# zongh5a/MDF-Net

Measured on AMD Instinct MI355X. Metric: views/sec at DTU 1600x1200x5-view x4-scale, higher is better.
Workload: dtype f32; 1 GPU; DTU eval 1600x1184 (1600x1200 cropped as load/dtueval.py:34), 5 views, 3 cost-volume stages + x2 refine = 4 output scales, hypotheses (48,24,8), batch 1 per rank, seeded random weights (pth/dtu_29.pth is not available offline); parallelism=views sharded over 1 rank(s), no collective

## Files before the change

### include/mdfnet_hip.h

```cpp
#ifndef MDFNET_HIP_H
#define MDFNET_HIP_H

#include <stdint.h>

#ifdef __cplusplus
extern "C" {
#endif

#define MDF_ABI_VERSION 1

#define MDF_OK 0
#define MDF_EARG (-1)
#define MDF_EUNSUPPORTED (-2)
#define MDF_EHIP (-3)

#define MDF_FEA_NCHW 0
#define MDF_FEA_NHWC 1
#define MDF_VOL_NCDHW 0
#define MDF_VOL_NDHWC 1

#define MDF_MAX_SRC_VIEWS 16
#define MDF_MAX_FUSE_VIEWS 1024

int mdf_abi_version(void);
const char* mdf_last_error(void);
const char* mdf_last_launch(void);
int mdf_release_stream(void* stream);

int mdf_homo_warp_fwd(const float* src_fea, int fea_layout, const float* proj, const float* hypos,
                      int hypos_per_pixel, float* out, int out_layout, int B, int C, int D, int h, int w,
                      void* stream);

int mdf_warp_corner_indices(const float* proj, const float* hypos, int hypos_per_pixel, int32_t* x0y0,
                            int B, int D, int h, int w, void* stream);

int mdf_warp_aggregate_vec_fwd(const float* ref_fea, const float* const* src_feas, int fea_layout,
                               const float* proj, const float* hypos, int hypos_per_pixel,
                               const float* w_params, float* cost, int cost_layout, int B, int C, int G,
                               int D, int h, int w, int n_src, void* stream);

int mdf_warp_aggregate_var_fwd(const float* ref_fea, const float* const* src_feas, int fea_layout,
                               const float* proj, const float* hypos, int hypos_per_pixel, float* cost,
                               int cost_layout, int B, int C, int D, int h, int w, int n_src, void* stream);

int mdf_conv3d_fwd(const float* x, const float* wpack, const float* alpha, const float* beta, const float* res,
                   float* y, int B, int Di, int Hi, int Wi, int Cin, int Cout, int stride, int transposed,
                   int relu, void* stream);

int64_t mdf_conv3d_packed_size(int Cin, int Cout);
int mdf_conv3d_pack_weights(const float* w, float* wpack, int Cin, int Cout, int transposed, void* stream);

int mdf_conv2d_fwd(const float* x, const float* wpack, const float* alpha, const float* beta, const float* res,
                   float res_scale, const float* res_up, float* y, int B, int H, int W, int Cin, int Cout, int ksize, int stride, int relu,
                   int planar_in, int pixel_shuffle2, void* stream);
int64_t mdf_conv_packed_size(int Cin, int Cout, int ntaps);
int mdf_conv_pack_weights(const float* w, float* wpack, int Cin, int Cout, int ntaps, void* stream);

int mdf_prob_softmax_regress_fwd(const float* x, const float* w, const float* hypos, int hypos_per_pixel,
                                 float* prob, float* depth, int B, int D, int h, int wd, int Cin, void* stream);
int mdf_prob_from_partials_fwd(const float* partials, const float* hypos, int hypos_per_pixel, float* prob, float* depth,
                               int B, int D, int h, int wd, void* stream);
int mdf_prob_fused_fwd(const float* x, const float* wpack, const float* hypos, int hypos_per_pixel, float* prob, float* depth,
                       int B, int D, int h, int wd, int Cin, void* stream);

int mdf_refine_tail_fwd(const float* x, const float* w1pack, const float* w2, const float* lo, const float* span, float* y,
                        int B, int H, int W, void* stream);

int mdf_conv2d_pair_fwd(const float* x, const float* w1pack, const float* alpha1, const float* beta1, const float* w2pack,
                        const float* alpha2, const float* beta2, float* y, int N, int H, int W, void* stream);

int mdf_conv1x1_heads_fwd(const float* x, int n_heads, const float* const* wpacks, const float* const* biases,
                          const float* const* res_ups, float* const* ys, const int* couts, int B, int H, int W, int Cin,
                          void* stream);

int mdf_refine_head_fwd(const float* depth, const float* lo, const float* span, const float* weight, float* y, int B, int H, int W,
                        void* stream);

int mdf_conv2d_res_pair_fwd(const float* x, const float* wa_pack, const float* wb_pack, float scale, float* y, int N, int H,
                            int W, void* stream);

int mdf_depth_regress_fwd(const float* prob, const float* hypos, int hypos_per_pixel, float* depth, int B, int D,
                          int h, int w, void* stream);

int mdf_confidence_fwd(const float* prob, float* conf, int64_t* idx_out, int B, int D, int h, int w, void* stream);
int mdf_confidence_up2_fwd(const float* prob, float* conf2, int B, int D, int h, int w, void* stream);
int mdf_range_affine_fwd(const float* x, const float* lo, const float* span, int mode, float* y, int B, long long n, void* stream);

int mdf_hypos_fit_fwd(int mode, const float* prob, const float* depth, const float* hypos, int hypos_per_pixel,
                      const float* fit_row, float* s_out, int B, int D, int h, int w, void* stream);
int mdf_hypos_from_fit_fwd(int mode, const float* s, const float* depth, const float* range, float log_thresh,
                           float* hypos_out, int B, int D_out, int h, int w, int upsample, void* stream);

int mdf_consistency_fuse_fwd(const float* depth_ref, const float* conf, const float* const* src_depths, const float* mats,
                             int n_src, int h, int w, float photo_threshold, int nconditions, float thre1, float thre2,
                             float* depth_avg, unsigned char* masks, unsigned short* view_masks, float* rep_out, void* stream);

long long mdf_consensus_fuse_workspace(int n, int h, int w);
int mdf_consensus_fuse_fwd(const float* depths, const unsigned char* colors, const float* cams, int n, int h, int w, float f,
                           float disp_thresh, int num_consistent, void* workspace, float* xyz, unsigned char* rgb,
                           long long capacity, int* view_counts, long long* total, void* stream);
int mdf_consensus_compact(void* workspace, int n, int h, int w, float* xyz, unsigned char* rgb, long long capacity, void* stream);

#define MDF_PCD_MAX_SOURCES 64
#define MDF_PCD_STEP_VIS1 1
#define MDF_PCD_STEP_FUSION 2
#define MDF_PCD_STEP_VIS2 3
#define MDF_PCD_STEP_AVE 4
#define MDF_PCD_STEP_VIS3 5
#define MDF_PCD_STEP_SEG 6
long long mdf_pcd_fuse_workspace(int n, int h, int w, int v);
int mdf_pcd_fuse_fwd(float* depths, unsigned char* masks, const float* cams, const int* srcs, int n, int h, int w, int v, int need,
                     int first_step, int last_step, void* workspace, int* view_counts, long long* total, void* stream);
int mdf_pcd_compact(const float* depths, const unsigned char* masks, const unsigned char* rgb, const float* cams, int n, int h,
                    int w, int v, void* workspace, float* xyz, unsigned char* rgb_out, float* dirs, long long capacity,
                    void* stream);

long long mdf_pts_index_workspace(long long n);
int mdf_pts_index_build(const double* pts, long long n, void* index, long long index_bytes, void* stream);
int mdf_pts_nn_dist(const void* index, long long n, long long index_bytes, const void* qindex, const double* queries, long long m,
                    long long qindex_bytes, const double* bb, double cap, double* dist, int* visits, void* stream);
long long mdf_pts_reduce_workspace(long long n);
int mdf_pts_reduce_count(const void* index, long long n, long long index_bytes, const int* rank, double dst, void* workspace,
                         long long ws_bytes, long long* edges, void* stream);
int mdf_pts_reduce(const void* index, long long n, long long index_bytes, const int* rank, double dst, void* workspace,
                   long long ws_bytes, int* csr, long long capacity, int resume, int max_rounds, unsigned char* keep, int* state,
                   void* stream);
int mdf_dtu_masks(const double* qdata, long long n, const unsigned char* obs_mask, int s1, int s2, int s3, const double* bb,
                  double res, unsigned char* in_mask, const double* qstl, long long m, const double* plane, unsigned char* above,
                  void* stream);


int mdf_bn_stats_fwd(const float* y, long long N, int C, int ngroups, double* sums, void* stream);
int mdf_bn_finalize_fwd(const double* sums, const float* gamma, const float* beta, float eps, float momentum, long long N,
                        int C, int ngroups, float* aux, float* running_mean, float* running_var,
                        long long* num_batches_tracked, int nslices, void* stream);
int mdf_bn_relu_apply_fwd(const float* y, const float* aux, const float* res, float* z, long long N, int C, int ngroups,
                          void* stream);
int mdf_bn_finalize_apply_fwd(const float* y, const double* sums, const float* gamma, const float* beta, float eps, float momentum,
                              const float* res, float* z, float* aux, float* running_mean, float* running_var,
                              long long* num_batches_tracked, long long N, int C, int ngroups, int nslices, void* stream);
int mdf_bn_relu_bwd_reduce(const float* dz, const float* y, const float* aux, long long N, int C, int ngroups, double* red,
                           void* stream);
int mdf_bn_relu_bwd(const float* dz, const float* y, const float* aux, const double* red, const float* gamma, long long N,
                    int C, int ngroups, float* dy, float* dgamma, float* dbeta, int nslices, void* stream);

int64_t mdf_conv3d_wgrad_workspace(int B, int Ds, int Hs, int Ws, int A, int Bc);
int mdf_conv3d_wgrad(const float* small_, const float* big, float* dw, float* workspace, int B, int Ds, int Hs, int Ws,
                     int A, int Bc, int stride, int accumulate, void* stream);
int64_t mdf_conv2d_wgrad_workspace(int B, int Hs, int Ws, int A, int Bc, int ksize);
int mdf_conv2d_wgrad(const float* small_, const float* big, float* dw, float* workspace, int B, int Hs, int Ws, int A, int Bc,
                     int ksize, int stride, int accumulate, void* stream);
int mdf_conv3d_wgrad_partial(const float* small_, const float* big, float* dw, float* workspace, int B, int Ds, int Hs, int Ws,
                             int A, int Bc, int stride, int* nslab_out, void* stream);
int mdf_conv2d_wgrad_partial(const float* small_, const float* big, float* dw, float* workspace, int B, int Hs, int Ws, int A, int Bc,
                             int ksize, int stride, int* nslab_out, void* stream);
int mdf_wgrad_sum_batch(const float* const* slabs, float* const* outs, const int* nslabs, const int* ns, int njobs, void* stream);
int mdf_wgrad_batch_begin(void);
int mdf_wgrad_batch_flush(void* stream);

int mdf_conv3d_train_fwd(const float* x, const float* wpack, const float* res, float* y, int B, int Di, int Hi, int Wi, int Cin,
                         int Cout, int stride, int transposed, int stat_mode, const float* stat_y, const float* stat_aux,
                         double* stat_out, int nslices, void* stream);
int mdf_conv2d_train_fwd(const float* x, const float* wpack, float* y, int B, int H, int W, int Cin_mem, int Cout, int ksize,
                         int stride, int planar_in, int stat_mode, const float* stat_y, const float* stat_aux, double* stat_out,
                         int nslices, int ngroups, void* stream);

int64_t mdf_pack_job_bytes(void);
int64_t mdf_pack_job_fill(void* jobs_host, int index, const float* src, float* dst, int is3d, int transposed, int mode,
                          int Cin, int Cout, int ntaps, int aux0, int aux1, int first_block);
int mdf_pack_batch(const void* jobs_dev, const int* block_job_dev, int nblocks, void* stream);

int mdf_upsample2_bilinear_bwd(const float* dfine, float* dcoarse, int B, int h, int w, int C, int accumulate, void* stream);

int mdf_prob_softmax_regress_bwd(const float* prob, const float* hypos, int hypos_per_pixel, const float* ddepth,
                                 const float* dprob, float* dlogit, int B, int D, int h, int w, void* stream);
int mdf_prob_conv_dgrad(const float* dlogit, const float* w, float* dx, int B, int D, int h, int wd, int C, void* stream);
int mdf_prob_conv_dgrad_stat(const float* dlogit, const float* w, float* dx, int B, int D, int h, int wd, int C, const float* stat_y,
                             const float* stat_aux, double* red, int nslices, void* stream);

int mdf_warp_aggregate_vec_train(int pass, const float* ref_fea, const float* const* src_feas, const float* proj,
                                 const float* hypos, int hypos_per_pixel, const float* par, const double* red_in,
                                 const float* dcost, float* cost, float* wsum, double* red_out, float* dref,
                                 float* const* dsrc, float* dcw, float* aux, int B, int C, int G, int D, int h, int w,
                                 int n_src, void* stream);
int mdf_aggregate_train_prepare(const float* cw, const float* w2, const float* b2, const float* gamma, long long n, int G,
                                int n_src, float* par, double* red, int nred, void* stream);
int mdf_aggregate_train_finalize(const double* red, const float* gamma, const float* beta, float eps, float momentum, long long n,
                                 int G, int n_src, float* par, float* running_mean, float* running_var,
                                 long long* num_batches_tracked, void* stream);
int mdf_aggregate_train_bwd_finalize(const float* dhalf, const double* red, int n_src, long long n_half, float* dsrc,
                                     float* dpar, const float* dref_acc, float* dref, long long n_ref, void* stream);

int mdf_masked_smooth_l1_reduce(const float* est, const float* gt, const void* floor_, int floor_f64, int floor_stride, int B,
                                long long per_batch, double* acc, void* stream);
int mdf_masked_smooth_l1_finalize(const double* acc, int nscales, float* loss, float* inv_count, void* stream);
int mdf_masked_smooth_l1_bwd(const float* est, const float* gt, const void* floor_, int floor_f64, int floor_stride, int B,
                             long long per_batch, const float* dloss, const float* inv_count, float* dest, void* stream);

int mdf_masked_smooth_l1_reduce_multi(const float* const* est, const float* const* gt, const long long* per_batch, int nscales,
                                      const void* floor_, int floor_f64, int floor_stride, int B, double* acc, void* stream);
int mdf_masked_smooth_l1_bwd_multi(const float* const* est, const float* const* gt, const long long* per_batch, int nscales,
                                   const void* floor_, int floor_f64, int floor_stride, int B, const float* dloss,
                                   const float* inv_count, float* const* dest, void* stream);

int mdf_fpn_compose_fwd(const float* O2, const float* O3, const float* L2, const float* b2, const float* L3, const float* b3,
                        int c2, int c3, int cm, float* comp, void* stream);
int mdf_fpn_compose_bwd(const float* O2, const float* O3, const float* L2, const float* b2, const float* L3, const float* b3,
                        const float* dA2, const float* dB3, const float* dA3, const float* W2, const float* W3,
                        const double* s2, const double* sc3, const double* s3, int c2, int c3, int cm, float* dO2, float* dO3,
                        float* dL2, float* dL3, float* db2, float* db3, void* stream);

int64_t mdf_adam_job_bytes(void);
int64_t mdf_adam_job_fill(void* jobs_host, int index, float* param, long long offset, long long n, int first_block);
int mdf_adam_step(const void* jobs_dev, const int* block_job_dev, int nblocks, const float* grads, float* exp_avg,
                  float* exp_avg_sq, float lr, float beta1, float beta2, float eps, float weight_decay, long long step,
                  void* stream);
int mdf_adam_step_hyper(const void* jobs_dev, const int* block_job_dev, int nblocks, const float* grads, float* exp_avg,
                        float* exp_avg_sq, const float* hyper_dev, float beta1, float beta2, float eps, float weight_decay,
                        void* stream);

#ifdef __cplusplus
}
#endif
#endif
```

### mdf-net_amd/csrc/conv1x1.hip

```cpp
#include <cstdlib>
#include "common.h"

namespace {

typedef float f32x4 __attribute__((ext_vector_type(4)));

struct P1 {
  const float* x;
  const float* wpack;
  const float* alpha;
  const float* beta;
  const float* res;
  const float* res_up;
  float* y;
  float res_scale;
  int relu;
  int Ho, Wo;
  long long npx;
  int n_runs;
};

struct PixBase { int img, oh, ow; };
__device__ __forceinline__ PixBase pix_base(unsigned first_px, int Ho, int Wo) {
  const unsigned rr = first_px / (unsigned)Wo, img = rr / (unsigned)Ho;
  return PixBase{(int)img, (int)(rr - img * (unsigned)Ho), (int)(first_px - rr * (unsigned)Wo)};
}
__device__ __forceinline__ void pix_at(const PixBase& b, int delta, int Ho, int Wo, int& img, int& oh, int& ow) {
  img = b.img; oh = b.oh; ow = b.ow + delta;
  while (ow >= Wo) {
    ow -= Wo;
    if (++oh == Ho) { oh = 0; ++img; }
  }
}

template <int CIN, int COUT>
__global__ __launch_bounds__(256) void conv1x1_kernel(const P1 p) {
  constexpr int NCH = CIN / 16, NT = COUT / 16;
  constexpr int U = (8 / NCH) < 1 ? 1 : 8 / NCH;
  const int lane = threadIdx.x & 63, q = lane >> 4, n16 = lane & 15;
  const int wave_g = blockIdx.x * 4 + (threadIdx.x >> 6), n_waves = gridDim.x * 4;

  float wr[NCH][NT][4];
#pragma unroll
  for (int ch = 0; ch < NCH; ++ch)
#pragma unroll
    for (int nt = 0; nt < NT; ++nt) {
      const float4 v = *reinterpret_cast<const float4*>(p.wpack + ((size_t)(ch * NT + nt) * 64 + lane) * 4);
      wr[ch][nt][0] = v.x; wr[ch][nt][1] = v.y; wr[ch][nt][2] = v.z; wr[ch][nt][3] = v.w;
    }
  float al[NT][4], be[NT][4];
#pragma unroll
  for (int nt = 0; nt < NT; ++nt)
#pragma unroll
    for (int k = 0; k < 4; ++k) {
      const int c = nt * 16 + 4 * q + k;
      al[nt][k] = p.alpha ? p.alpha[c] : 1.f;
      be[nt][k] = p.beta ? p.beta[c] : 0.f;
    }

  for (int run = wave_g; run < p.n_runs; run += n_waves) {
    const long long px0 = (long long)run * (U * 16) + n16;
    float4 xb[U][NCH];
#pragma unroll
    for (int u = 0; u < U; ++u) {
      const long long px = px0 + u * 16;
#pragma unroll
      for (int ch = 0; ch < NCH; ++ch)
        xb[u][ch] = (px < p.npx) ? *reinterpret_cast<const float4*>(p.x + px * CIN + ch * 16 + 4 * q) : make_float4(0.f, 0.f, 0.f, 0.f);
    }
    PixBase pb{0, 0, 0};
    if (p.res_up) pb = pix_base((unsigned)run * (U * 16), p.Ho, p.Wo);
#pragma unroll
    for (int u = 0; u < U; ++u) {
      const long long px = px0 + u * 16;
      f32x4 acc[NT];
#pragma unroll
      for (int nt = 0; nt < NT; ++nt) acc[nt] = (f32x4){0.f, 0.f, 0.f, 0.f};
#pragma unroll
      for (int ch = 0; ch < NCH; ++ch) {
        const float b4[4] = {xb[u][ch].x, xb[u][ch].y, xb[u][ch].z, xb[u][ch].w};
#pragma unroll
        for (int s = 0; s < 4; ++s)
#pragma unroll
          for (int nt = 0; nt < NT; ++nt) acc[nt] = __builtin_amdgcn_mfma_f32_16x16x4f32(wr[ch][nt][s], b4[s], acc[nt], 0, 0, 0);
      }
      if (px >= p.npx) continue;
      int oh = 0, ow = 0, img = 0;
      if (p.res_up) pix_at(pb, u * 16 + n16, p.Ho, p.Wo, img, oh, ow);
#pragma unroll
      for (int nt = 0; nt < NT; ++nt) {
        const int c0 = nt * 16 + 4 * q;
        float o[4];
#pragma unroll
        for (int k = 0; k < 4; ++k) {
          o[k] = acc[nt][k] * al[nt][k] + be[nt][k];
          if (p.relu) o[k] = fmaxf(o[k], 0.f);
        }
        if (p.res_up) {
          const int Hh = p.Ho >> 1, Wh = p.Wo >> 1;
          float sy = ((float)oh + 0.5f) * 0.5f - 0.5f; sy = sy < 0.f ? 0.f : sy;
          float sx = ((float)ow + 0.5f) * 0.5f - 0.5f; sx = sx < 0.f ? 0.f : sx;
          const int y0 = (int)sy, x0 = (int)sx;
          const int y1 = y0 + (y0 < Hh - 1), x1 = x0 + (x0 < Wh - 1);
          const float ly1 = sy - (float)y0, ly0 = 1.f - ly1, lx1 = sx - (float)x0, lx0 = 1.f - lx1;
          const float* base = p.res_up + (size_t)img * Hh * Wh * COUT + c0;
          const float4 v00 = *reinterpret_cast<const float4*>(base + ((size_t)y0 * Wh + x0) * COUT);
          const float4 v01 = *reinterpret_cast<const float4*>(base + ((size_t)y0 * Wh + x1) * COUT);
          const float4 v10 = *reinterpret_cast<const float4*>(base + ((size_t)y1 * Wh + x0) * COUT);
          const float4 v11 = *reinterpret_cast<const float4*>(base + ((size_t)y1 * Wh + x1) * COUT);
          const float w00 = ly0 * lx0, w01 = ly0 * lx1, w10 = ly1 * lx0, w11 = ly1 * lx1;
          o[0] = __fmaf_rn(w11, v11.x, __fmaf_rn(w10, v10.x, __fmaf_rn(w00, v00.x, w01 * v01.x))) + o[0];
          o[1] = __fmaf_rn(w11, v11.y, __fmaf_rn(w10, v10.y, __fmaf_rn(w00, v00.y, w01 * v01.y))) + o[1];
          o[2] = __fmaf_rn(w11, v11.z, __fmaf_rn(w10, v10.z, __fmaf_rn(w00, v00.z, w01 * v01.z))) + o[2];
          o[3] = __fmaf_rn(w11, v11.w, __fmaf_rn(w10, v10.w, __fmaf_rn(w00, v00.w, w01 * v01.w))) + o[3];
        }
        const size_t oi = (size_t)px * COUT + c0;
        if (p.res) {
          const float4 rv = *reinterpret_cast<const float4*>(p.res + oi);
          o[0] = rv.x + o[0] * p.res_scale; o[1] = rv.y + o[1] * p.res_scale;
          o[2] = rv.z + o[2] * p.res_scale; o[3] = rv.w + o[3] * p.res_scale;
        }
        *reinterpret_cast<float4*>(p.y + oi) = make_float4(o[0], o[1], o[2], o[3]);
      }
    }
  }
}

struct P1M {
  const float* x;
  const float* wpack[3];
  const float* beta[3];
  const float* res_up[3];
  float* y[3];
  int Ho, Wo;
  long long npx;
  int n_runs;
};

template <int CIN, int C0, int C1, int C2, int U>
__global__ __launch_bounds__(256) void conv1x1_heads_kernel(const P1M p) {
  constexpr int NCH = CIN / 16;
  constexpr int N0 = C0 / 16, N1 = C1 / 16, N2 = C2 / 16, NT = N0 + N1 + N2;
  const int lane = threadIdx.x & 63, q = lane >> 4, n16 = lane & 15;
  const int wave_g = blockIdx.x * 4 + (threadIdx.x >> 6), n_waves = gridDim.x * 4;
  auto head_of = [](int nt) { return nt < N0 ? 0 : (nt < N0 + N1 ? 1 : 2); };
  auto first_of = [](int h) { return h == 0 ? 0 : (h == 1 ? N0 : N0 + N1); };
  auto cout_of = [](int h) { return h == 0 ? C0 : (h == 1 ? C1 : C2); };

  constexpr bool WLDS = (NCH * NT * 4 > 64);
  __shared__ __attribute__((aligned(16))) float wsm[WLDS ? NCH * NT * 64 * 4 : 4];
  float wr[WLDS ? 1 : NCH][WLDS ? 1 : NT][4];
  float be[NT][4];
#pragma unroll
  for (int nt = 0; nt < NT; ++nt) {
    const int h = head_of(nt), lt = nt - first_of(h), nth = cout_of(h) / 16;
#pragma unroll
    for (int ch = 0; ch < NCH; ++ch) {
      if constexpr (WLDS) {
        if (threadIdx.x < 64)
          *reinterpret_cast<float4*>(wsm + ((ch * NT + nt) * 64 + lane) * 4) = *reinterpret_cast<const float4*>(p.wpack[h] + ((size_t)(ch * nth + lt) * 64 + lane) * 4);
      } else {
        const float4 v = *reinterpret_cast<const float4*>(p.wpack[h] + ((size_t)(ch * nth + lt) * 64 + lane) * 4);
        wr[ch][nt][0] = v.x; wr[ch][nt][1] = v.y; wr[ch][nt][2] = v.z; wr[ch][nt][3] = v.w;
      }
    }
#pragma unroll
    for (int k = 0; k < 4; ++k) be[nt][k] = p.beta[h] ? p.beta[h][lt * 16 + 4 * q + k] : 0.f;
  }
  if constexpr (WLDS) __syncthreads();

  for (int run = wave_g; run < p.n_runs; run += n_waves) {
    const long long px0 = (long long)run * (U * 16) + n16;
    float4 xb[U][NCH];
#pragma unroll
    for (int u = 0; u < U; ++u) {
      const long long px = px0 + u * 16;
#pragma unroll
      for (int ch = 0; ch < NCH; ++ch)
        xb[u][ch] = (px < p.npx) ? *reinterpret_cast<const float4*>(p.x + px * CIN + ch * 16 + 4 * q) : make_float4(0.f, 0.f, 0.f, 0.f);
    }
    const PixBase pb = pix_base((unsigned)run * (U * 16), p.Ho, p.Wo);
#pragma unroll
    for (int u = 0; u < U; ++u) {
      const long long px = px0 + u * 16;
      f32x4 acc[NT];
#pragma unroll
      for (int nt = 0; nt < NT; ++nt) acc[nt] = (f32x4){0.f, 0.f, 0.f, 0.f};
#pragma unroll
      for (int ch = 0; ch < NCH; ++ch) {
        const float b4[4] = {xb[u][ch].x, xb[u][ch].y, xb[u][ch].z, xb[u][ch].w};
        if constexpr (WLDS) {
          asm volatile("" ::: "memory");
#pragma unroll
          for (int nt = 0; nt < NT; ++nt) {
            const float4 wv = *reinterpret_cast<const float4*>(wsm + ((ch * NT + nt) * 64 + lane) * 4);
            const float w4[4] = {wv.x, wv.y, wv.z, wv.w};
#pragma unroll
            for (int s = 0; s < 4; ++s) acc[nt] = __builtin_amdgcn_mfma_f32_16x16x4f32(w4[s], b4[s], acc[nt], 0, 0, 0);
          }
        } else {
#pragma unroll
          for (int s = 0; s < 4; ++s)
#pragma unroll
            for (int nt = 0; nt < NT; ++nt) acc[nt] = __builtin_amdgcn_mfma_f32_16x16x4f32(wr[ch][nt][s], b4[s], acc[nt], 0, 0, 0);
        }
      }
      if (px >= p.npx) continue;
      int img, oh, ow;
      pix_at(pb, u * 16 + n16, p.Ho, p.Wo, img, oh, ow);
      const int Hh = p.Ho >> 1, Wh = p.Wo >> 1;
      float sy = ((float)oh + 0.5f) * 0.5f - 0.5f; sy = sy < 0.f ? 0.f : sy;
      float sx = ((float)ow + 0.5f) * 0.5f - 0.5f; sx = sx < 0.f ? 0.f : sx;
      const int y0 = (int)sy, x0 = (int)sx;
      const int y1 = y0 + (y0 < Hh - 1), x1 = x0 + (x0 < Wh - 1);
      const float ly1 = sy - (float)y0, ly0 = 1.f - ly1, lx1 = sx - (float)x0, lx0 = 1.f - lx1;
      const float w00 = ly0 * lx0, w01 = ly0 * lx1, w10 = ly1 * lx0, w11 = ly1 * lx1;
#pragma unroll
      for (int nt = 0; nt < NT; ++nt) {
        const int h = head_of(nt), co = cout_of(h), c0 = (nt - first_of(h)) * 16 + 4 * q;
        float o[4];
#pragma unroll
        for (int k = 0; k < 4; ++k) o[k] = acc[nt][k] * 1.0f + be[nt][k];
        if (p.res_up[h]) {
          const float* base = p.res_up[h] + (size_t)img * Hh * Wh * co + c0;
          const float4 v00 = *reinterpret_cast<const float4*>(base + ((size_t)y0 * Wh + x0) * co);
          const float4 v01 = *reinterpret_cast<const float4*>(base + ((size_t)y0 * Wh + x1) * co);
          const float4 v10 = *reinterpret_cast<const float4*>(base + ((size_t)y1 * Wh + x0) * co);
          const float4 v11 = *reinterpret_cast<const float4*>(base + ((size_t)y1 * Wh + x1) * co);
          o[0] = __fmaf_rn(w11, v11.x, __fmaf_rn(w10, v10.x, __fmaf_rn(w00, v00.x, w01 * v01.x))) + o[0];
          o[1] = __fmaf_rn(w11, v11.y, __fmaf_rn(w10, v10.y, __fmaf_rn(w00, v00.y, w01 * v01.y))) + o[1];
          o[2] = __fmaf_rn(w11, v11.z, __fmaf_rn(w10, v10.z, __fmaf_rn(w00, v00.z, w01 * v01.z))) + o[2];
          o[3] = __fmaf_rn(w11, v11.w, __fmaf_rn(w10, v10.w, __fmaf_rn(w00, v00.w, w01 * v01.w))) + o[3];
        }
        *reinterpret_cast<float4*>(p.y[h] + (size_t)px * co + c0) = make_float4(o[0], o[1], o[2], o[3]);
      }
    }
  }
}

template <int CIN, int C0, int C1, int C2, int U>
int launch_heads(P1M& p, hipStream_t st) {
  const long long runs = (p.npx + U * 16 - 1) / (U * 16);
  if (runs > 0x7fffffff) return mdf::fail(MDF_EARG, "conv1x1 heads: too many pixels");
  p.n_runs = (int)runs;
  long long blocks = (runs + 3) / 4;
  if (blocks > 256 * 8) blocks = 256 * 8;
  hipLaunchKernelGGL((conv1x1_heads_kernel<CIN, C0, C1, C2, U>), dim3((unsigned)blocks), dim3(256), 0, st, p);
  return mdf::check_launch("conv1x1_heads_kernel");
}

template <int CIN, int COUT>
int launch_1x1(P1& p, hipStream_t st) {
  constexpr int NCH = CIN / 16;
  constexpr int U = (8 / NCH) < 1 ? 1 : 8 / NCH;
  const long long runs = (p.npx + U * 16 - 1) / (U * 16);
  if (runs > 0x7fffffff) return mdf::fail(MDF_EARG, "conv1x1: too many pixels");
  p.n_runs = (int)runs;
  long long blocks = (runs + 3) / 4;
  int cap = 256 * 8;
  if (const char* e = getenv("MDF_CONV1X1_BLOCKS")) { if (atoi(e) > 0) cap = atoi(e); }
  if (blocks > cap) blocks = cap;
  hipLaunchKernelGGL((conv1x1_kernel<CIN, COUT>), dim3((unsigned)blocks), dim3(256), 0, st, p);
  return mdf::check_launch("conv1x1_kernel");
}

}

#define C1_CASE(ci, co) \
  if (Cin == ci && Cout == co) return launch_1x1<ci, co>(p, (hipStream_t)stream);

int mdf_conv1x1_dispatch(const float* x, const float* wpack, const float* alpha, const float* beta, const float* res, float res_scale,
                         const float* res_up, float* y, int B, int H, int W, int Cin, int Cout, int relu, void* stream) {
  if (const char* e = getenv("MDF_CONV1X1")) { if (atoi(e) == 0) return MDF_EUNSUPPORTED; }
  P1 p{};
  p.x = x; p.wpack = wpack; p.alpha = alpha; p.beta = beta; p.res = res; p.res_up = res_up; p.y = y;
  p.res_scale = res_scale; p.relu = relu; p.Ho = H; p.Wo = W; p.npx = (long long)B * H * W;
  if (p.npx >= (1ll << 31) - 256) return MDF_EUNSUPPORTED;
  C1_CASE(16, 16) C1_CASE(16, 32) C1_CASE(16, 64) C1_CASE(32, 16) C1_CASE(32, 32) C1_CASE(32, 64)
  return MDF_EUNSUPPORTED;
}

extern "C" int mdf_conv1x1_heads_fwd(const float* x, int n_heads, const float* const* wpacks, const float* const* biases,
                                     const float* const* res_ups, float* const* ys, const int* couts, int B, int H, int W, int Cin,
                                     void* stream) {
  MDF_REQUIRE(x && wpacks && biases && res_ups && ys && couts, "null pointer argument");
  MDF_REQUIRE(n_heads == 2 || n_heads == 3, "n_heads=%d not in {2,3}", n_heads);
  MDF_REQUIRE(B > 0 && H > 0 && W > 0, "bad shape");
  P1M p{};
  p.x = x; p.Ho = H; p.Wo = W; p.npx = (long long)B * H * W;
  bool any_up = false;
  for (int h = 0; h < n_heads; ++h) {
    MDF_REQUIRE(wpacks[h] && ys[h], "head %d: null weights or output", h);
    p.wpack[h] = wpacks[h]; p.beta[h] = biases[h]; p.res_up[h] = res_ups[h]; p.y[h] = ys[h];
    any_up = any_up || res_ups[h];
    MDF_REQUIRE((long long)p.npx * couts[h] < (1ll << 31) && (long long)p.npx * Cin < (1ll << 31), "map too large for 32-bit offsets");
  }
  MDF_REQUIRE(!any_up || (H % 2 == 0 && W % 2 == 0), "upsample-add needs even H and W");
  hipStream_t st = (hipStream_t)stream;
  if (Cin == 64 && n_heads == 3 && couts[0] == 64 && couts[1] == 32 && couts[2] == 16) return launch_heads<64, 64, 32, 16, 1>(p, st);
  if (Cin == 32 && n_heads == 2 && couts[0] == 32 && couts[1] == 16) return launch_heads<32, 32, 16, 0, 1>(p, st);
  return mdf::fail(MDF_EUNSUPPORTED, "conv1x1 heads: Cin=%d with %d heads is not built (64 -> 64/32/16, 32 -> 32/16)", Cin, n_heads);
}
```

### mdf-net_amd/csrc/warp_aggregate.hip

```cpp
#include <cstdlib>
#include "warp_common.h"

namespace {

enum Mode { kWarp = 0, kVec = 1, kVar = 2 };

struct Params {
  const float* ref;
  const float* src[MDF_MAX_SRC_VIEWS];
  const float* proj;
  const float* hypos;
  const float* wpar;
  float* out;
  Geom g;
  int B, D, n_src, hypos_per_pixel, out_ndhwc, dchunk, nblk_x;
};

template <int C, int MODE>
__global__ __launch_bounds__(kThreads) void warp_kernel(const Params p) {
  constexpr int LPP = C / 4;
  constexpr int PPB = kThreads / LPP;
  extern __shared__ __attribute__((aligned(16))) char smem[];
  TapEntry* tab = reinterpret_cast<TapEntry*>(smem);

  const int hw = p.g.h * p.g.w;
  const int b = blockIdx.y;
  const PixTile<PPB> pt((int)mdf::xcd_remap(blockIdx.x, p.nblk_x), p.g.w);
  const int tid = threadIdx.x;
  const int pl = tid / LPP;
  const int sub = tid % LPP;
  bool live;
  const int pix = pt.pix(pl, p.g.w, p.g.h, live);
  const int G = C / 2;

  float r[4] = {0.f, 0.f, 0.f, 0.f};
  float cw0 = 0.f, cw1 = 0.f, alpha = 0.f, beta = 0.f, w2 = 0.f, b2 = 0.f;
  if (MODE != kWarp) {
    const float4 rv = *reinterpret_cast<const float4*>(p.ref + ((size_t)b * hw + pix) * C + 4 * sub);
    if (MODE == kVec) {
      softmax2(rv.x, rv.y, r[0], r[1]);
      softmax2(rv.z, rv.w, r[2], r[3]);
      r[0] -= r[1];
      r[2] -= r[3];
      cw0 = p.wpar[2 * sub];
      cw1 = p.wpar[2 * sub + 1];
      alpha = p.wpar[G];
      beta = p.wpar[G + 1];
      w2 = p.wpar[G + 2];
      b2 = p.wpar[G + 3];
    } else {
      r[0] = rv.x; r[1] = rv.y; r[2] = rv.z; r[3] = rv.w;
    }
  }
  const size_t map_stride = (size_t)hw * C;
  const unsigned lane_b = 16u * (unsigned)sub;

  const int npair = PPB * p.n_src;
  const bool fixed_pair = (kThreads % npair) == 0;
  const int pa_pair = tid % npair, pa_grp = tid / npair, pa_ngrp = kThreads / npair;
  const int pa_pl = pa_pair % PPB, pa_v = pa_pair / PPB;
  bool pa_live;
  const int pa_pix = pt.pix(pa_pl, p.g.w, p.g.h, pa_live);
  PixelRay ray{};
  if (fixed_pair) {
    const int yy = pa_pix / p.g.w, xx = pa_pix - yy * p.g.w;
    ray = warp_ray(p.proj + ((size_t)pa_v * p.B + b) * 12, (float)xx, (float)yy);
  }

  for (int d0 = 0; d0 < p.D; d0 += p.dchunk) {
    const int nd = min(p.dchunk, p.D - d0);
    if (fixed_pair) {
      for (int ed = pa_grp; ed < nd; ed += pa_ngrp) {
        const int d = d0 + ed;
        const float dep = p.hypos_per_pixel ? p.hypos[((size_t)b * p.D + d) * hw + pa_pix] : p.hypos[(size_t)b * p.D + d];
        float ix, iy;
        warp_position_ray(ray, dep, p.g, ix, iy);
        TapEntry t;
        make_taps(ix, iy, p.g, C, t);
        tab[(ed * p.n_src + pa_v) * PPB + pa_pl] = t;
      }
    } else {
      const int nent = nd * p.n_src * PPB;
      for (int e = tid; e < nent; e += kThreads) {
        const int epl = e % PPB;
        const int ev = (e / PPB) % p.n_src;
        const int ed = e / (PPB * p.n_src);
        bool elive;
        const int epix = pt.pix(epl, p.g.w, p.g.h, elive);
        const int yy = epix / p.g.w, xx = epix - yy * p.g.w;
        const float* m = p.proj + ((size_t)ev * p.B + b) * 12;
        const int d = d0 + ed;
        const float dep = p.hypos_per_pixel ? p.hypos[((size_t)b * p.D + d) * hw + epix] : p.hypos[(size_t)b * p.D + d];
        float ix, iy;
        warp_position(m, (float)xx, (float)yy, dep, p.g, ix, iy);
        TapEntry t;
        make_taps(ix, iy, p.g, C, t);
        tab[e] = t;
      }
    }
    __syncthreads();
    for (int dd = 0; dd < nd; ++dd) {
      const int d = d0 + dd;
      float acc[4] = {0.f, 0.f, 0.f, 0.f};
      float acc2[4] = {0.f, 0.f, 0.f, 0.f};
      float wsum = 0.f;
      if (MODE == kVar) {
#pragma unroll
        for (int k = 0; k < 4; ++k) { acc[k] = r[k]; acc2[k] = r[k] * r[k]; }
      }
      for (int v = 0; v < p.n_src; ++v) {
        const TapEntry t = tab[(dd * p.n_src + v) * PPB + pl];
        const char* sb = reinterpret_cast<const char*>(p.src[v] + (size_t)b * map_stride);
        const float4 nw = *reinterpret_cast<const float4*>(sb + ((unsigned)t.off[0] * 4u + lane_b));
        const float4 ne = *reinterpret_cast<const float4*>(sb + ((unsigned)t.off[1] * 4u + lane_b));
        const float4 sw = *reinterpret_cast<const float4*>(sb + ((unsigned)t.off[2] * 4u + lane_b));
        const float4 se = *reinterpret_cast<const float4*>(sb + ((unsigned)t.off[3] * 4u + lane_b));
        float val[4];
        val[0] = __fmaf_rn(se.x, t.wt[3], __fmaf_rn(sw.x, t.wt[2], __fmaf_rn(ne.x, t.wt[1], __fmul_rn(nw.x, t.wt[0]))));
        val[1] = __fmaf_rn(se.y, t.wt[3], __fmaf_rn(sw.y, t.wt[2], __fmaf_rn(ne.y, t.wt[1], __fmul_rn(nw.y, t.wt[0]))));
        val[2] = __fmaf_rn(se.z, t.wt[3], __fmaf_rn(sw.z, t.wt[2], __fmaf_rn(ne.z, t.wt[1], __fmul_rn(nw.z, t.wt[0]))));
        val[3] = __fmaf_rn(se.w, t.wt[3], __fmaf_rn(sw.w, t.wt[2], __fmaf_rn(ne.w, t.wt[1], __fmul_rn(nw.w, t.wt[0]))));
        if (MODE == kWarp) {
#pragma unroll
          for (int k = 0; k < 4; ++k) acc[k] = val[k];
        } else if (MODE == kVec) {
          const float sim0 = __fmaf_rn(softmax2_p0(val[0], val[1]), r[0], r[1]);
          const float sim1 = __fmaf_rn(softmax2_p0(val[2], val[3]), r[2], r[3]);
          const float z = pixel_sum<LPP>(__fmaf_rn(cw0, sim0, cw1 * sim1));
          const float u = __fmaf_rn(fmaxf(__fmaf_rn(z, alpha, beta), 0.0f), w2, b2);
          const float wv = __builtin_amdgcn_rcpf(1.0f + __builtin_amdgcn_exp2f(-u * kLog2e));
          wsum += wv;
          acc[0] += wv * sim0;
          acc[1] += wv * sim1;
        } else {
          const float mx = pixel_max<LPP>(fmaxf(fmaxf(val[0], val[1]), fmaxf(val[2], val[3])));
          float e[4];
#pragma unroll
          for (int k = 0; k < 4; ++k) e[k] = expf(val[k] - mx);
          const float den = pixel_sum<LPP>((e[0] + e[1]) + (e[2] + e[3]));
#pragma unroll
          for (int k = 0; k < 4; ++k) {
            const float pr = e[k] / den;
            acc[k] += pr;
            acc2[k] += pr * pr;
          }
        }
      }
      if (!live) continue;
      const size_t vox = ((size_t)b * p.D + d) * hw + pix;
      if (MODE == kVec) {
        const float o0 = acc[0] / wsum, o1 = acc[1] / wsum;
        if (p.out_ndhwc) {
          { typedef float f2v __attribute__((ext_vector_type(2))); f2v ov = {o0, o1}; __builtin_nontemporal_store(ov, reinterpret_cast<f2v*>(p.out + vox * G + 2 * sub)); }
        } else {
          const size_t cs = (size_t)p.D * hw;
          float* o = p.out + ((size_t)b * G * p.D + d) * hw + pix;
          o[(size_t)(2 * sub) * cs] = o0;
          o[(size_t)(2 * sub + 1) * cs] = o1;
        }
      } else {
        float o[4];
        if (MODE == kVar) {
          const float n = (float)(p.n_src + 1);
#pragma unroll
          for (int k = 0; k < 4; ++k) {
            const float mean = acc[k] / n;
            o[k] = acc2[k] / n - mean * mean;
          }
        } else {
#pragma unroll
          for (int k = 0; k < 4; ++k) o[k] = acc[k];
        }
        if (p.out_ndhwc) {
          *reinterpret_cast<float4*>(p.out + vox * C + 4 * sub) = make_float4(o[0], o[1], o[2], o[3]);
        } else {
          const size_t cs = (size_t)p.D * hw;
          float* op = p.out + ((size_t)b * C * p.D + d) * hw + pix;
#pragma unroll
          for (int k = 0; k < 4; ++k) op[(size_t)(4 * sub + k) * cs] = o[k];
        }
      }
    }
    __syncthreads();
  }
}

#ifndef MDF_VEC8_MIN_BLOCKS
#define MDF_VEC8_MIN_BLOCKS 1
#endif
#ifndef MDF_VEC8_TAB
#define MDF_VEC8_TAB 1024
#endif
template <int C>
__global__ __launch_bounds__(kThreads, MDF_VEC8_MIN_BLOCKS) void warp_vec8_kernel(const Params p) {
  constexpr int LPP = C / 8;
  constexpr int PPB = kThreads / LPP;
  constexpr int G = C / 2;
  extern __shared__ __attribute__((aligned(16))) char smem[];
  TapEntry* tab = reinterpret_cast<TapEntry*>(smem);
  const int hw = p.g.h * p.g.w;
  const int b = blockIdx.y;
  const PixTile<PPB> pt((int)mdf::xcd_remap(blockIdx.x, p.nblk_x), p.g.w);
  const int tid = threadIdx.x;
  const int pl = tid / LPP, sub = tid % LPP;
  bool live;
  const int pix = pt.pix(pl, p.g.w, p.g.h, live);

  float rd[2][2], r1[2][2], cw[2][2];
#pragma unroll
  for (int j = 0; j < 2; ++j) {
    const float4 rv = *reinterpret_cast<const float4*>(p.ref + ((size_t)b * hw + pix) * C + 8 * sub + 4 * j);
    float a0, a1, b0, b1;
    softmax2(rv.x, rv.y, a0, a1);
    softmax2(rv.z, rv.w, b0, b1);
    rd[j][0] = a0 - a1; r1[j][0] = a1;
    rd[j][1] = b0 - b1; r1[j][1] = b1;
    cw[j][0] = p.wpar[2 * (2 * sub + j)];
    cw[j][1] = p.wpar[2 * (2 * sub + j) + 1];
  }
  const float alpha = p.wpar[G], beta = p.wpar[G + 1], w2 = p.wpar[G + 2], b2 = p.wpar[G + 3];
  const size_t map_stride = (size_t)hw * C;
  const unsigned lane_b = 32u * (unsigned)sub;

  const int npair = PPB * p.n_src;
  const bool few = (npair <= kThreads) && (kThreads % npair) == 0;
  const bool two = (npair == 2 * kThreads);
  const int pa_ngrp = few ? kThreads / npair : 1, pa_grp = few ? tid / npair : 0;
  PixelRay ray[2];
  int pa_pl[2], pa_v[2], pa_pix[2];
#pragma unroll
  for (int k = 0; k < 2; ++k) {
    const int pair = (few ? tid % npair : tid) + k * kThreads;
    pa_pl[k] = pair % PPB; pa_v[k] = min(pair / PPB, p.n_src - 1);
    bool pa_live;
    pa_pix[k] = pt.pix(pa_pl[k], p.g.w, p.g.h, pa_live);
    const int yy = pa_pix[k] / p.g.w, xx = pa_pix[k] - yy * p.g.w;
    ray[k] = warp_ray(p.proj + ((size_t)pa_v[k] * p.B + b) * 12, (float)xx, (float)yy);
  }

  for (int d0 = 0; d0 < p.D; d0 += p.dchunk) {
    const int nd = min(p.dchunk, p.D - d0);
    if (few || two) {
#pragma unroll
      for (int k = 0; k < 2; ++k) {
        if (k == 1 && !two) break;
        for (int ed = pa_grp; ed < nd; ed += pa_ngrp) {
          const int d = d0 + ed;
          const float dep = p.hypos_per_pixel ? p.hypos[((size_t)b * p.D + d) * hw + pa_pix[k]] : p.hypos[(size_t)b * p.D + d];
          float ix, iy;
          warp_position_ray(ray[k], dep, p.g, ix, iy);
          TapEntry t;
          make_taps(ix, iy, p.g, C, t);
          tab[(ed * p.n_src + pa_v[k]) * PPB + pa_pl[k]] = t;
        }
      }
    } else {
      const int nent = nd * p.n_src * PPB;
      for (int e = tid; e < nent; e += kThreads) {
        const int epl = e % PPB;
        const int ev = (e / PPB) % p.n_src;
        const int ed = e / (PPB * p.n_src);
        bool elive;
        const int epix = pt.pix(epl, p.g.w, p.g.h, elive);
        const int yy = epix / p.g.w, xx = epix - yy * p.g.w;
        const float* m = p.proj + ((size_t)ev * p.B + b) * 12;
        const int d = d0 + ed;
        const float dep = p.hypos_per_pixel ? p.hypos[((size_t)b * p.D + d) * hw + epix] : p.hypos[(size_t)b * p.D + d];
        float ix, iy;
        warp_position(m, (float)xx, (float)yy, dep, p.g, ix, iy);
        TapEntry t;
        make_taps(ix, iy, p.g, C, t);
        tab[e] = t;
      }
    }
    __syncthreads();
    for (int dd = 0; dd < nd; ++dd) {
      float acc[2][2] = {{0.f, 0.f}, {0.f, 0.f}};
      float wsum = 0.f;
      for (int v = 0; v < p.n_src; ++v) {
        const TapEntry t = tab[(dd * p.n_src + v) * PPB + pl];
        const char* sb = reinterpret_cast<const char*>(p.src[v] + (size_t)b * map_stride);
        float sim[2][2], part[2];
#pragma unroll
        for (int j = 0; j < 2; ++j) {
          const unsigned lb = lane_b + 16u * j;
          const float4 nw = *reinterpret_cast<const float4*>(sb + ((unsigned)t.off[0] * 4u + lb));
          const float4 ne = *reinterpret_cast<const float4*>(sb + ((unsigned)t.off[1] * 4u + lb));
          const float4 sw = *reinterpret_cast<const float4*>(sb + ((unsigned)t.off[2] * 4u + lb));
          const float4 se = *reinterpret_cast<const float4*>(sb + ((unsigned)t.off[3] * 4u + lb));
          const float v0 = __fmaf_rn(se.x, t.wt[3], __fmaf_rn(sw.x, t.wt[2], __fmaf_rn(ne.x, t.wt[1], __fmul_rn(nw.x, t.wt[0]))));
          const float v1 = __fmaf_rn(se.y, t.wt[3], __fmaf_rn(sw.y, t.wt[2], __fmaf_rn(ne.y, t.wt[1], __fmul_rn(nw.y, t.wt[0]))));
          const float v2 = __fmaf_rn(se.z, t.wt[3], __fmaf_rn(sw.z, t.wt[2], __fmaf_rn(ne.z, t.wt[1], __fmul_rn(nw.z, t.wt[0]))));
          const float v3 = __fmaf_rn(se.w, t.wt[3], __fmaf_rn(sw.w, t.wt[2], __fmaf_rn(ne.w, t.wt[1], __fmul_rn(nw.w, t.wt[0]))));
          sim[j][0] = __fmaf_rn(softmax2_p0(v0, v1), rd[j][0], r1[j][0]);
          sim[j][1] = __fmaf_rn(softmax2_p0(v2, v3), rd[j][1], r1[j][1]);
          part[j] = __fmaf_rn(cw[j][0], sim[j][0], cw[j][1] * sim[j][1]);
        }
        const float z = pixel_sum<LPP>(part[0] + part[1]);
        const float u = __fmaf_rn(fmaxf(__fmaf_rn(z, alpha, beta), 0.0f), w2, b2);
        const float wv = __builtin_amdgcn_rcpf(1.0f + __builtin_amdgcn_exp2f(-u * kLog2e));
        wsum += wv;
#pragma unroll
        for (int j = 0; j < 2; ++j) {
          acc[j][0] += wv * sim[j][0];
          acc[j][1] += wv * sim[j][1];
        }
      }
      if (!live) continue;
      const size_t vox = ((size_t)b * p.D + d0 + dd) * hw + pix;
      const float o0 = acc[0][0] / wsum, o1 = acc[0][1] / wsum, o2 = acc[1][0] / wsum, o3 = acc[1][1] / wsum;
      if (p.out_ndhwc) {
        { typedef float f4v __attribute__((ext_vector_type(4))); f4v ov = {o0, o1, o2, o3}; __builtin_nontemporal_store(ov, reinterpret_cast<f4v*>(p.out + vox * G + 4 * sub)); }
      } else {
        const size_t cs = (size_t)p.D * hw;
        float* o = p.out + ((size_t)b * G * p.D + d0 + dd) * hw + pix;
        o[(size_t)(4 * sub) * cs] = o0;
        o[(size_t)(4 * sub + 1) * cs] = o1;
        o[(size_t)(4 * sub + 2) * cs] = o2;
        o[(size_t)(4 * sub + 3) * cs] = o3;
      }
    }
    __syncthreads();
  }
}

template <int C>
int launch_vec8(Params& p, hipStream_t st) {
  constexpr int ppb = kThreads / (C / 8);
  p.nblk_x = PixTile<ppb>::blocks(p.g.w, p.g.h);
  int dch = MDF_VEC8_TAB / (p.n_src * ppb);
  if (dch < 1) dch = 1;
  if (dch > p.D) dch = p.D;
  p.dchunk = dch;
  const size_t lds = (size_t)dch * p.n_src * ppb * sizeof(TapEntry);
  if (lds > 64 * 1024) return MDF_EUNSUPPORTED;
  hipLaunchKernelGGL((warp_vec8_kernel<C>), dim3(p.nblk_x, p.B), dim3(kThreads), lds, st, p);
  return mdf::check_launch("warp_vec8_kernel");
}

struct WinDesc {
  int off;
  int xmin, ymin, ww;
};

template <int C>
__global__ __launch_bounds__(kThreads) void warp_vec_win_kernel(const Params p, int pool_floats) {
  constexpr int LPP = C / 4;
  constexpr int PPB = kThreads / LPP;
  constexpr int G = C / 2;
  extern __shared__ __attribute__((aligned(16))) char smem[];
  TapXY* tab = reinterpret_cast<TapXY*>(smem);
  float* pool = reinterpret_cast<float*>(smem + (size_t)p.dchunk * p.n_src * PPB * sizeof(TapXY));
  __shared__ int bb[MDF_MAX_SRC_VIEWS][4];
  __shared__ WinDesc wd[MDF_MAX_SRC_VIEWS];

  const int hw = p.g.h * p.g.w;
  const int W = p.g.w;
  const int b = blockIdx.y;
  const int tile = (int)mdf::xcd_remap(blockIdx.x, p.nblk_x);
  const int pix0 = tile * PPB;
  const int tid = threadIdx.x;
  const int pl = tid / LPP, sub = tid % LPP;
  const int pix = min(pix0 + pl, hw - 1);
  const bool live = (pix0 + pl) < hw;

  float r[4];
  {
    const float4 rv = *reinterpret_cast<const float4*>(p.ref + ((size_t)b * hw + pix) * C + 4 * sub);
    softmax2(rv.x, rv.y, r[0], r[1]);
    softmax2(rv.z, rv.w, r[2], r[3]);
    r[0] -= r[1];
    r[2] -= r[3];
  }
  const float cw0 = p.wpar[2 * sub], cw1 = p.wpar[2 * sub + 1];
  const float alpha = p.wpar[G], beta = p.wpar[G + 1], w2 = p.wpar[G + 2], b2 = p.wpar[G + 3];
  const size_t map_stride = (size_t)hw * C;

  for (int d0 = 0; d0 < p.D; d0 += p.dchunk) {
    const int nd = min(p.dchunk, p.D - d0);
    if (tid < 4 * p.n_src) bb[tid >> 2][tid & 3] = (tid & 1) ? INT32_MIN : INT32_MAX;
    __syncthreads();
    const int nent = nd * p.n_src * PPB;
    for (int e = tid; e < nent; e += kThreads) {
      const int epl = e % PPB;
      const int ev = (e / PPB) % p.n_src;
      const int ed = e / (PPB * p.n_src);
      const int epix = min(pix0 + epl, hw - 1);
      const int yy = epix / W, xx = epix - yy * W;
      const float* m = p.proj + ((size_t)ev * p.B + b) * 12;
      const int d = d0 + ed;
      const float dep = p.hypos_per_pixel ? p.hypos[((size_t)b * p.D + d) * hw + epix] : p.hypos[(size_t)b * p.D + d];
      float ix, iy;
      warp_position(m, (float)xx, (float)yy, dep, p.g, ix, iy);
      TapXY t;
      tap_weights_corners(ix, iy, p.g, t.wt, t.xa, t.xb, t.ya, t.yb);
      tab[e] = t;
      atomicMin(&bb[ev][0], t.xa);
      atomicMax(&bb[ev][1], t.xb);
      atomicMin(&bb[ev][2], t.ya);
      atomicMax(&bb[ev][3], t.yb);
    }
    __syncthreads();
    if (tid == 0) {
      int used = 0;
      for (int v = 0; v < p.n_src; ++v) {
        const int ww = bb[v][1] - bb[v][0] + 1, wh = bb[v][3] - bb[v][2] + 1;
        const long long need = (long long)ww * wh * C;
        WinDesc w_;
        w_.xmin = bb[v][0]; w_.ymin = bb[v][2]; w_.ww = ww;
        if (need <= pool_floats - used) { w_.off = used; used += (int)need; } else { w_.off = -1; }
        wd[v] = w_;
      }
    }
    __syncthreads();
    for (int v = 0; v < p.n_src; ++v) {
      const WinDesc w_ = wd[v];
      if (w_.off < 0) continue;
      const int wh = bb[v][3] - bb[v][2] + 1;
      const int row4 = w_.ww * (C / 4);
      const float* sv = p.src[v] + (size_t)b * map_stride;
      for (int wy = 0; wy < wh; ++wy) {
        const float4* grow = reinterpret_cast<const float4*>(sv + ((size_t)(w_.ymin + wy) * W + w_.xmin) * C);
        float4* lrow = reinterpret_cast<float4*>(pool + w_.off) + wy * row4;
        for (int j = tid; j < row4; j += kThreads) lrow[j] = grow[j];
      }
    }
    __syncthreads();

    for (int dd = 0; dd < nd; ++dd) {
      float acc0 = 0.f, acc1 = 0.f, wsum = 0.f;
      for (int v = 0; v < p.n_src; ++v) {
        const TapXY t = tab[(dd * p.n_src + v) * PPB + pl];
        const WinDesc w_ = wd[v];
        float4 nw, ne, sw, se;
        if (w_.off >= 0) {
          const float* lp = pool + w_.off + 4 * sub;
          const int ra = (t.ya - w_.ymin) * w_.ww, rb = (t.yb - w_.ymin) * w_.ww, ca = t.xa - w_.xmin, cb = t.xb - w_.xmin;
          nw = *reinterpret_cast<const float4*>(lp + (ra + ca) * C);
          ne = *reinterpret_cast<const float4*>(lp + (ra + cb) * C);
          sw = *reinterpret_cast<const float4*>(lp + (rb + ca) * C);
          se = *reinterpret_cast<const float4*>(lp + (rb + cb) * C);
        } else {
          const float* sp = p.src[v] + (size_t)b * map_stride + 4 * sub;
          nw = *reinterpret_cast<const float4*>(sp + (size_t)(t.ya * W + t.xa) * C);
          ne = *reinterpret_cast<const float4*>(sp + (size_t)(t.ya * W + t.xb) * C);
          sw = *reinterpret_cast<const float4*>(sp + (size_t)(t.yb * W + t.xa) * C);
          se = *reinterpret_cast<const float4*>(sp + (size_t)(t.yb * W + t.xb) * C);
        }
        const float v0 = __fmaf_rn(se.x, t.wt[3], __fmaf_rn(sw.x, t.wt[2], __fmaf_rn(ne.x, t.wt[1], __fmul_rn(nw.x, t.wt[0]))));
        const float v1 = __fmaf_rn(se.y, t.wt[3], __fmaf_rn(sw.y, t.wt[2], __fmaf_rn(ne.y, t.wt[1], __fmul_rn(nw.y, t.wt[0]))));
        const float v2 = __fmaf_rn(se.z, t.wt[3], __fmaf_rn(sw.z, t.wt[2], __fmaf_rn(ne.z, t.wt[1], __fmul_rn(nw.z, t.wt[0]))));
        const float v3 = __fmaf_rn(se.w, t.wt[3], __fmaf_rn(sw.w, t.wt[2], __fmaf_rn(ne.w, t.wt[1], __fmul_rn(nw.w, t.wt[0]))));
        const float sim0 = __fmaf_rn(softmax2_p0(v0, v1), r[0], r[1]);
        const float sim1 = __fmaf_rn(softmax2_p0(v2, v3), r[2], r[3]);
        const float z = pixel_sum<LPP>(__fmaf_rn(cw0, sim0, cw1 * sim1));
        const float u = __fmaf_rn(fmaxf(__fmaf_rn(z, alpha, beta), 0.0f), w2, b2);
        const float wv = __builtin_amdgcn_rcpf(1.0f + __builtin_amdgcn_exp2f(-u * kLog2e));
        wsum += wv;
        acc0 += wv * sim0;
        acc1 += wv * sim1;
      }
      if (!live) continue;
      const size_t vox = ((size_t)b * p.D + d0 + dd) * hw + pix;
      const float o0 = acc0 / wsum, o1 = acc1 / wsum;
      if (p.out_ndhwc) {
        *reinterpret_cast<float2*>(p.out + vox * G + 2 * sub) = make_float2(o0, o1);
      } else {
        const size_t cs = (size_t)p.D * hw;
        float* o = p.out + ((size_t)b * G * p.D + d0 + dd) * hw + pix;
        o[(size_t)(2 * sub) * cs] = o0;
        o[(size_t)(2 * sub + 1) * cs] = o1;
      }
    }
    __syncthreads();
  }
}

template <int C>
int launch_win(Params& p, hipStream_t st) {
  constexpr int ppb = kThreads / (C / 4);
  const int hw = p.g.h * p.g.w;
  p.nblk_x = (hw + ppb - 1) / ppb;
  int dch = 512 / (p.n_src * ppb);
  if (const char* e = getenv("MDF_WARP_DCHUNK")) { if (atoi(e) > 0) dch = atoi(e); }
  if (dch < 1) dch = 1;
  if (dch > p.D) dch = p.D;
  p.dchunk = dch;
  int pool_kb = 64;
  if (const char* e = getenv("MDF_WARP_POOL_KB")) { if (atoi(e) > 0) pool_kb = atoi(e); }
  const size_t tab_bytes = (size_t)dch * p.n_src * ppb * sizeof(TapXY);
  const size_t lds = tab_bytes + (size_t)pool_kb * 1024;
  if (lds > 150 * 1024) return MDF_EUNSUPPORTED;
  static bool attr_done[64] = {};
  int dev_id = 0;
  (void)hipGetDevice(&dev_id);
  if (dev_id < 0 || dev_id >= 64 || !attr_done[dev_id]) {
    hipError_t e = hipFuncSetAttribute(reinterpret_cast<const void*>(&warp_vec_win_kernel<C>), hipFuncAttributeMaxDynamicSharedMemorySize, 150 * 1024);
    if (e != hipSuccess) return mdf::fail(MDF_EHIP, "hipFuncSetAttribute(dynamic LDS): %s", hipGetErrorString(e));
    if (dev_id >= 0 && dev_id < 64) attr_done[dev_id] = true;
  }
  hipLaunchKernelGGL((warp_vec_win_kernel<C>), dim3(p.nblk_x, p.B), dim3(kThreads), lds, st, p, pool_kb * 256);
  return mdf::check_launch("warp_vec_win_kernel");
}

__global__ void corner_index_kernel(const float* __restrict__ proj, const float* __restrict__ hypos, int per_pixel,
                                    int32_t* __restrict__ out, Geom g, int B, int D) {
  const int hw = g.h * g.w;
  const size_t n = (size_t)B * D * hw;
  for (size_t i = (size_t)blockIdx.x * blockDim.x + threadIdx.x; i < n; i += (size_t)gridDim.x * blockDim.x) {
    const int pix = (int)(i % hw);
    const int d = (int)((i / hw) % D);
    const int b = (int)(i / ((size_t)hw * D));
    const int yy = pix / g.w, xx = pix - yy * g.w;
    const float dep = per_pixel ? hypos[i] : hypos[(size_t)b * D + d];
    float ix, iy;
    warp_position(proj + (size_t)b * 12, (float)xx, (float)yy, dep, g, ix, iy);
    const float lim = 1073741824.0f;
    const bool fin = (fabsf(ix) <= 3.0e38f) && (fabsf(iy) <= 3.0e38f);
    int32_t x0 = INT32_MIN, y0 = INT32_MIN;
    if (fin) {
      x0 = (int32_t)fminf(fmaxf(floorf(ix), -lim), lim);
      y0 = (int32_t)fminf(fmaxf(floorf(iy), -lim), lim);
    }
    out[2 * i] = x0;
    out[2 * i + 1] = y0;
  }
}

template <int MODE>
int launch(Params& p, int C, hipStream_t st) {
  const int lpp = C / 4, ppb = kThreads / lpp;
  p.nblk_x = (C == 64) ? PixTile<16>::blocks(p.g.w, p.g.h) : (C == 32) ? PixTile<32>::blocks(p.g.w, p.g.h) : PixTile<64>::blocks(p.g.w, p.g.h);
  int dch = 512 / (p.n_src * ppb);
  if (dch < 1) dch = 1;
  if (dch > p.D) dch = p.D;
  p.dchunk = dch;
  const size_t lds = (size_t)dch * p.n_src * ppb * sizeof(TapEntry);
  dim3 grid(p.nblk_x, p.B), block(kThreads);
  switch (C) {
    case 64: hipLaunchKernelGGL((warp_kernel<64, MODE>), grid, block, lds, st, p); break;
    case 32: hipLaunchKernelGGL((warp_kernel<32, MODE>), grid, block, lds, st, p); break;
    case 16: hipLaunchKernelGGL((warp_kernel<16, MODE>), grid, block, lds, st, p); break;
    default: return mdf::fail(MDF_EUNSUPPORTED, "warp kernels are built for C in {16,32,64}, got %d", C);
  }
  return mdf::check_launch("warp_kernel");
}

int check_common(const void* a, const void* b, const void* c, const void* d, int fea_layout, int B, int C, int D, int h,
                 int w) {
  MDF_REQUIRE(a && b && c && d, "null pointer argument");
  MDF_REQUIRE(B > 0 && D > 0 && h > 1 && w > 1, "bad shape B=%d D=%d h=%d w=%d", B, D, h, w);
  MDF_REQUIRE((long long)h * w * C < (1ll << 30), "feature map too large for 32-bit byte offsets");
  if (fea_layout != MDF_FEA_NHWC)
    return mdf::fail(MDF_EUNSUPPORTED, "feature layout %d not supported (kernels gather NHWC taps)", fea_layout);
  if (C != 16 && C != 32 && C != 64)
    return mdf::fail(MDF_EUNSUPPORTED, "C=%d not supported (built for 16, 32, 64)", C);
  return MDF_OK;
}

}

extern "C" int mdf_homo_warp_fwd(const float* src_fea, int fea_layout, const float* proj, const float* hypos,
                                 int hypos_per_pixel, float* out, int out_layout, int B, int C, int D, int h, int w,
                                 void* stream) {
  if (int rc = check_common(src_fea, proj, hypos, out, fea_layout, B, C, D, h, w)) return rc;
  Params p{};
  p.src[0] = src_fea;
  p.proj = proj;
  p.hypos = hypos;
  p.out = out;
  p.g = make_geom(h, w);
  p.B = B; p.D = D; p.n_src = 1; p.hypos_per_pixel = hypos_per_pixel; p.out_ndhwc = (out_layout == MDF_VOL_NDHWC);
  return launch<kWarp>(p, C, (hipStream_t)stream);
}

extern "C" int mdf_warp_corner_indices(const float* proj, const float* hypos, int hypos_per_pixel, int32_t* x0y0,
                                       int B, int D, int h, int w, void* stream) {
  MDF_REQUIRE(proj && hypos && x0y0, "null pointer argument");
  MDF_REQUIRE(B > 0 && D > 0 && h > 1 && w > 1, "bad shape");
  const size_t n = (size_t)B * D * h * w;
  const int grid = (int)((n + 255) / 256 < 4096 ? (n + 255) / 256 : 4096);
  hipLaunchKernelGGL(corner_index_kernel, dim3(grid), dim3(256), 0, (hipStream_t)stream, proj, hypos, hypos_per_pixel,
                     x0y0, make_geom(h, w), B, D);
  return mdf::check_launch("corner_index_kernel");
}

extern "C" int mdf_warp_aggregate_vec_fwd(const float* ref_fea, const float* const* src_feas, int fea_layout,
                                          const float* proj, const float* hypos, int hypos_per_pixel,
                                          const float* w_params, float* cost, int cost_layout, int B, int C, int G,
                                          int D, int h, int w, int n_src, void* stream) {
  if (int rc = check_common(ref_fea, proj, hypos, cost, fea_layout, B, C, D, h, w)) return rc;
  MDF_REQUIRE(src_feas && w_params, "null pointer argument");
  MDF_REQUIRE(n_src >= 1 && n_src <= MDF_MAX_SRC_VIEWS, "n_src=%d out of range [1,%d]", n_src, MDF_MAX_SRC_VIEWS);
  if (G * 2 != C) return mdf::fail(MDF_EUNSUPPORTED, "only C/G == 2 is built (C=%d, G=%d)", C, G);
  Params p{};
  p.ref = ref_fea;
  for (int v = 0; v < n_src; ++v) {
    MDF_REQUIRE(src_feas[v], "src_feas[%d] is null", v);
    p.src[v] = src_feas[v];
  }
  p.proj = proj; p.hypos = hypos; p.wpar = w_params; p.out = cost;
  p.g = make_geom(h, w);
  p.B = B; p.D = D; p.n_src = n_src; p.hypos_per_pixel = hypos_per_pixel; p.out_ndhwc = (cost_layout == MDF_VOL_NDHWC);
  const char* we = getenv("MDF_WARP_WINDOW");
  if (we && atoi(we) != 0) {
    int rc = MDF_EUNSUPPORTED;
    if (C == 64) rc = launch_win<64>(p, (hipStream_t)stream);
    else if (C == 32) rc = launch_win<32>(p, (hipStream_t)stream);
    else if (C == 16) rc = launch_win<16>(p, (hipStream_t)stream);
    if (rc != MDF_EUNSUPPORTED) return rc;
  }
  {
    const char* e8 = getenv("MDF_WARP_VEC8");
    if (!e8 || atoi(e8) != 0) {
      int rc = MDF_EUNSUPPORTED;
      if (C == 64) rc = launch_vec8<64>(p, (hipStream_t)stream);
      else if (C == 32) rc = launch_vec8<32>(p, (hipStream_t)stream);
      else if (C == 16 && e8 && atoi(e8) == 2) rc = launch_vec8<16>(p, (hipStream_t)stream);
      if (rc != MDF_EUNSUPPORTED) return rc;
    }
  }
  return launch<kVec>(p, C, (hipStream_t)stream);
}

extern "C" int mdf_warp_aggregate_var_fwd(const float* ref_fea, const float* const* src_feas, int fea_layout,
                                          const float* proj, const float* hypos, int hypos_per_pixel, float* cost,
                                          int cost_layout, int B, int C, int D, int h, int w, int n_src, void* stream) {
  if (int rc = check_common(ref_fea, proj, hypos, cost, fea_layout, B, C, D, h, w)) return rc;
  MDF_REQUIRE(src_feas, "null pointer argument");
  MDF_REQUIRE(n_src >= 1 && n_src <= MDF_MAX_SRC_VIEWS, "n_src=%d out of range [1,%d]", n_src, MDF_MAX_SRC_VIEWS);
  Params p{};
  p.ref = ref_fea;
  for (int v = 0; v < n_src; ++v) {
    MDF_REQUIRE(src_feas[v], "src_feas[%d] is null", v);
    p.src[v] = src_feas[v];
  }
  p.proj = proj; p.hypos = hypos; p.out = cost;
  p.g = make_geom(h, w);
  p.B = B; p.D = D; p.n_src = n_src; p.hypos_per_pixel = hypos_per_pixel; p.out_ndhwc = (cost_layout == MDF_VOL_NDHWC);
  return launch<kVar>(p, C, (hipStream_t)stream);
}
```

### mdf-net_amd/mdfnet_hip/__init__.py

```python
import ctypes
import os
import threading

import torch

_PKG = os.path.dirname(os.path.abspath(__file__))
LIB_PATH = os.environ.get("MDF_HIP_LIB") or os.path.join(_PKG, "libmdfnet_hip.so")
ABI_VERSION = 1

_lib = None
_lock = threading.Lock()

c_fp = ctypes.c_void_p
c_int = ctypes.c_int
c_i64 = ctypes.c_int64

SIGNATURES = {
    "mdf_abi_version": (c_int, []),
    "mdf_last_error": (ctypes.c_char_p, []),
    "mdf_last_launch": (ctypes.c_char_p, []),
    "mdf_release_stream": (c_int, [c_fp]),
    "mdf_homo_warp_fwd": (c_int, [c_fp, c_int, c_fp, c_fp, c_int, c_fp, c_int] + [c_int] * 5 + [c_fp]),
    "mdf_warp_corner_indices": (c_int, [c_fp, c_fp, c_int, c_fp] + [c_int] * 4 + [c_fp]),
    "mdf_warp_aggregate_vec_fwd": (c_int, [c_fp, ctypes.POINTER(c_fp), c_int, c_fp, c_fp, c_int, c_fp, c_fp, c_int]
                                   + [c_int] * 7 + [c_fp]),
    "mdf_warp_aggregate_var_fwd": (c_int, [c_fp, ctypes.POINTER(c_fp), c_int, c_fp, c_fp, c_int, c_fp, c_int]
                                   + [c_int] * 6 + [c_fp]),
    "mdf_conv3d_fwd": (c_int, [c_fp] * 6 + [c_int] * 9 + [c_fp]),
    "mdf_conv3d_packed_size": (c_i64, [c_int, c_int]),
    "mdf_conv3d_pack_weights": (c_int, [c_fp, c_fp, c_int, c_int, c_int, c_fp]),
    "mdf_conv2d_fwd": (c_int, [c_fp] * 5 + [ctypes.c_float, c_fp, c_fp] + [c_int] * 10 + [c_fp]),
    "mdf_conv2d_pair_fwd": (c_int, [c_fp] * 8 + [c_int] * 3 + [c_fp]),
    "mdf_conv1x1_heads_fwd": (c_int, [c_fp, c_int, ctypes.POINTER(c_fp), ctypes.POINTER(c_fp), ctypes.POINTER(c_fp), ctypes.POINTER(c_fp),
                                      ctypes.POINTER(c_int)] + [c_int] * 4 + [c_fp]),
    "mdf_refine_head_fwd": (c_int, [c_fp] * 5 + [c_int] * 3 + [c_fp]),
    "mdf_conv2d_res_pair_fwd": (c_int, [c_fp] * 3 + [ctypes.c_float, c_fp] + [c_int] * 3 + [c_fp]),
    "mdf_refine_tail_fwd": (c_int, [c_fp] * 6 + [c_int] * 3 + [c_fp]),
    "mdf_conv_packed_size": (c_i64, [c_int, c_int, c_int]),
    "mdf_conv_pack_weights": (c_int, [c_fp, c_fp, c_int, c_int, c_int, c_fp]),
    "mdf_prob_softmax_regress_fwd": (c_int, [c_fp, c_fp, c_fp, c_int, c_fp, c_fp] + [c_int] * 5 + [c_fp]),
    "mdf_prob_from_partials_fwd": (c_int, [c_fp, c_fp, c_int, c_fp, c_fp] + [c_int] * 4 + [c_fp]),
    "mdf_prob_fused_fwd": (c_int, [c_fp, c_fp, c_fp, c_int, c_fp, c_fp] + [c_int] * 5 + [c_fp]),
    "mdf_depth_regress_fwd": (c_int, [c_fp, c_fp, c_int, c_fp] + [c_int] * 4 + [c_fp]),
    "mdf_confidence_fwd": (c_int, [c_fp, c_fp, c_fp] + [c_int] * 4 + [c_fp]),
    "mdf_confidence_up2_fwd": (c_int, [c_fp, c_fp] + [c_int] * 4 + [c_fp]),
    "mdf_range_affine_fwd": (c_int, [c_fp, c_fp, c_fp, c_int, c_fp, c_int, c_i64, c_fp]),
    "mdf_hypos_fit_fwd": (c_int, [c_int, c_fp, c_fp, c_fp, c_int, c_fp, c_fp] + [c_int] * 4 + [c_fp]),
    "mdf_consistency_fuse_fwd": (c_int, [c_fp, c_fp, ctypes.POINTER(c_fp), c_fp, c_int, c_int, c_int, ctypes.c_float, c_int,
                                         ctypes.c_float, ctypes.c_float, c_fp, c_fp, c_fp, c_fp, c_fp]),
    "mdf_consensus_fuse_workspace": (c_i64, [c_int, c_int, c_int]),
    "mdf_consensus_fuse_fwd": (c_int, [c_fp, c_fp, c_fp, c_int, c_int, c_int, ctypes.c_float, ctypes.c_float, c_int, c_fp, c_fp, c_fp,
                                       c_i64, c_fp, c_fp, c_fp]),
    "mdf_consensus_compact": (c_int, [c_fp, c_int, c_int, c_int, c_fp, c_fp, c_i64, c_fp]),
    "mdf_pcd_fuse_workspace": (c_i64, [c_int, c_int, c_int, c_int]),
    "mdf_pcd_fuse_fwd": (c_int, [c_fp, c_fp, c_fp, c_fp] + [c_int] * 7 + [c_fp, c_fp, c_fp, c_fp]),
    "mdf_pcd_compact": (c_int, [c_fp, c_fp, c_fp, c_fp] + [c_int] * 4 + [c_fp, c_fp, c_fp, c_fp, c_i64, c_fp]),
    "mdf_pts_index_workspace": (c_i64, [c_i64]),
    "mdf_pts_index_build": (c_int, [c_fp, c_i64, c_fp, c_i64, c_fp]),
    "mdf_pts_nn_dist": (c_int, [c_fp, c_i64, c_i64, c_fp, c_fp, c_i64, c_i64, ctypes.POINTER(ctypes.c_double), ctypes.c_double, c_fp,
                                c_fp, c_fp]),
    "mdf_pts_reduce_workspace": (c_i64, [c_i64]),
    "mdf_pts_reduce_count": (c_int, [c_fp, c_i64, c_i64, c_fp, ctypes.c_double, c_fp, c_i64, c_fp, c_fp]),
    "mdf_pts_reduce": (c_int, [c_fp, c_i64, c_i64, c_fp, ctypes.c_double, c_fp, c_i64, c_fp, c_i64, c_int, c_int, c_fp, c_fp, c_fp]),
    "mdf_dtu_masks": (c_int, [c_fp, c_i64, c_fp, c_int, c_int, c_int, ctypes.POINTER(ctypes.c_double), ctypes.c_double, c_fp, c_fp,
                              c_i64, ctypes.POINTER(ctypes.c_double), c_fp, c_fp]),
    "mdf_bn_stats_fwd": (c_int, [c_fp, c_i64, c_int, c_int, c_fp, c_fp]),
    "mdf_bn_finalize_fwd": (c_int, [c_fp, c_fp, c_fp, ctypes.c_float, ctypes.c_float, c_i64, c_int, c_int, c_fp, c_fp, c_fp, c_fp, c_int, c_fp]),
    "mdf_bn_relu_apply_fwd": (c_int, [c_fp, c_fp, c_fp, c_fp, c_i64, c_int, c_int, c_fp]),
    "mdf_bn_finalize_apply_fwd": (c_int, [c_fp, c_fp, c_fp, c_fp, ctypes.c_float, ctypes.c_float, c_fp, c_fp, c_fp, c_fp, c_fp, c_fp, c_i64, c_int, c_int, c_int, c_fp]),
    "mdf_bn_relu_bwd_reduce": (c_int, [c_fp, c_fp, c_fp, c_i64, c_int, c_int, c_fp, c_fp]),
    "mdf_bn_relu_bwd": (c_int, [c_fp, c_fp, c_fp, c_fp, c_fp, c_i64, c_int, c_int, c_fp, c_fp, c_fp, c_int, c_fp]),
    "mdf_conv3d_wgrad_workspace": (c_i64, [c_int] * 6),
    "mdf_conv3d_wgrad": (c_int, [c_fp] * 4 + [c_int] * 8 + [c_fp]),
    "mdf_conv3d_train_fwd": (c_int, [c_fp] * 4 + [c_int] * 9 + [c_fp] * 3 + [c_int, c_fp]),
    "mdf_conv2d_train_fwd": (c_int, [c_fp] * 3 + [c_int] * 9 + [c_fp] * 3 + [c_int, c_int, c_fp]),
    "mdf_conv3d_wgrad_partial": (c_int, [c_fp] * 4 + [c_int] * 7 + [ctypes.POINTER(c_int), c_fp]),
    "mdf_conv2d_wgrad_partial": (c_int, [c_fp] * 4 + [c_int] * 7 + [ctypes.POINTER(c_int), c_fp]),
    "mdf_wgrad_sum_batch": (c_int, [ctypes.POINTER(c_fp), ctypes.POINTER(c_fp), ctypes.POINTER(c_int), ctypes.POINTER(c_int), c_int, c_fp]),
    "mdf_wgrad_batch_begin": (c_int, []),
    "mdf_wgrad_batch_flush": (c_int, [c_fp]),
    "mdf_conv2d_wgrad_workspace": (c_i64, [c_int] * 6),
    "mdf_conv2d_wgrad": (c_int, [c_fp] * 4 + [c_int] * 8 + [c_fp]),
    "mdf_pack_job_bytes": (c_i64, []),
    "mdf_pack_job_fill": (c_i64, [c_fp, c_int, c_fp, c_fp] + [c_int] * 9),
    "mdf_pack_batch": (c_int, [c_fp, c_fp, c_int, c_fp]),
    "mdf_upsample2_bilinear_bwd": (c_int, [c_fp, c_fp] + [c_int] * 5 + [c_fp]),
    "mdf_prob_softmax_regress_bwd": (c_int, [c_fp, c_fp, c_int, c_fp, c_fp, c_fp] + [c_int] * 4 + [c_fp]),
    "mdf_prob_conv_dgrad": (c_int, [c_fp, c_fp, c_fp] + [c_int] * 5 + [c_fp]),
    "mdf_prob_conv_dgrad_stat": (c_int, [c_fp, c_fp, c_fp] + [c_int] * 5 + [c_fp, c_fp, c_fp, c_int, c_fp]),
    "mdf_warp_aggregate_vec_train": (c_int, [c_int, c_fp, ctypes.POINTER(c_fp), c_fp, c_fp, c_int, c_fp, c_fp, c_fp, c_fp, c_fp, c_fp,
                                             c_fp, ctypes.POINTER(c_fp), c_fp, c_fp] + [c_int] * 7 + [c_fp]),
    "mdf_aggregate_train_prepare": (c_int, [c_fp] * 4 + [c_i64, c_int, c_int, c_fp, c_fp, c_int, c_fp]),
    "mdf_aggregate_train_finalize": (c_int, [c_fp] * 3 + [ctypes.c_float, ctypes.c_float, c_i64, c_int, c_int] + [c_fp] * 5),
    "mdf_aggregate_train_bwd_finalize": (c_int, [c_fp, c_fp, c_int, c_i64, c_fp, c_fp, c_fp, c_fp, c_i64, c_fp]),
    "mdf_masked_smooth_l1_reduce": (c_int, [c_fp, c_fp, c_fp, c_int, c_int, c_int, c_i64, c_fp, c_fp]),
    "mdf_masked_smooth_l1_finalize": (c_int, [c_fp, c_int, c_fp, c_fp, c_fp]),
    "mdf_masked_smooth_l1_bwd": (c_int, [c_fp, c_fp, c_fp, c_int, c_int, c_int, c_i64, c_fp, c_fp, c_fp, c_fp]),
    "mdf_masked_smooth_l1_reduce_multi": (c_int, [ctypes.POINTER(c_fp), ctypes.POINTER(c_fp), ctypes.POINTER(c_i64), c_int, c_fp, c_int, c_int, c_int, c_fp, c_fp]),
    "mdf_masked_smooth_l1_bwd_multi": (c_int, [ctypes.POINTER(c_fp), ctypes.POINTER(c_fp), ctypes.POINTER(c_i64), c_int, c_fp, c_int, c_int, c_int, c_fp, c_fp,
                                               ctypes.POINTER(c_fp), c_fp]),
    "mdf_fpn_compose_fwd": (c_int, [c_fp] * 6 + [c_int] * 3 + [c_fp, c_fp]),
    "mdf_fpn_compose_bwd": (c_int, [c_fp] * 14 + [c_int] * 3 + [c_fp] * 7),
    "mdf_adam_job_bytes": (c_i64, []),
    "mdf_adam_job_fill": (c_i64, [c_fp, c_int, c_fp, c_i64, c_i64, c_int]),
    "mdf_adam_step": (c_int, [c_fp, c_fp, c_int, c_fp, c_fp, c_fp] + [ctypes.c_float] * 5 + [c_i64, c_fp]),
    "mdf_adam_step_hyper": (c_int, [c_fp, c_fp, c_int, c_fp, c_fp, c_fp, c_fp] + [ctypes.c_float] * 4 + [c_fp]),
    "mdf_hypos_from_fit_fwd": (c_int, [c_int, c_fp, c_fp, c_fp, ctypes.c_float, c_fp] + [c_int] * 5 + [c_fp]),
}


class MdfHipError(RuntimeError):
    pass


def lib():
    global _lib
    if _lib is None:
        with _lock:
            if _lib is None:
                if not os.path.exists(LIB_PATH):
                    raise MdfHipError(
                        f"{LIB_PATH} not found: the HIP extension is not built and there is no fallback path. "
                        "Run `python -m mdfnet_hip.build` (needs hipcc, --offload-arch=gfx950).")
                h = ctypes.CDLL(LIB_PATH)
                for name, (res, args) in SIGNATURES.items():
                    fn = getattr(h, name)
                    fn.restype = res
                    fn.argtypes = args
                if h.mdf_abi_version() != ABI_VERSION:
                    raise MdfHipError(f"ABI version mismatch: library {h.mdf_abi_version()}, binding {ABI_VERSION}")
                _lib = h
    return _lib


def check(rc, what):
    if rc != 0:
        msg = lib().mdf_last_error().decode("utf-8", "replace")
        raise MdfHipError(f"{what} failed with code {rc}: {msg}")


def pcd_fuse(*args, **kwargs):
    from .ops import pcd_fuse as _pcd_fuse
    return _pcd_fuse(*args, **kwargs)


def dtu_eval_scan(*args, **kwargs):
    from .ops import dtu_eval_scan as _dtu_eval_scan
    return _dtu_eval_scan(*args, **kwargs)
```

### mdf-net_amd/mdfnet_hip/kernel_families.py

```python
import re

MFMA_CONV = "mfma_conv"
WARP = "warp_aggregate"
WARP_TRAIN = "aggregate_train_passes"
WARP_SCATTER = "aggregate_scatter"
WGRAD = "wgrad"
BN = "batchnorm_train"
PROB = "prob_head"
HEADS = "heads"
FILTER = "consistency_filter"
POINT_EVAL = "point_eval"
CONTROL = "control"

KERNEL_FAMILY = {
    "conv_lds_kernel": MFMA_CONV, "conv3d_kernel": MFMA_CONV, "conv3d_wlds_kernel": MFMA_CONV, "convtr_all_kernel": MFMA_CONV, "convtr_cls_kernel": MFMA_CONV, "conv_pair_kernel": MFMA_CONV, "conv_pair_valu_kernel": MFMA_CONV,
    "conv1x1_kernel": MFMA_CONV, "conv1x1_heads_kernel": MFMA_CONV, "refine_tail_kernel": MFMA_CONV, "prob_fused_kernel": MFMA_CONV, "res_pair_kernel": MFMA_CONV,
    "wino3d_kernel": MFMA_CONV, "wino2d_kernel": MFMA_CONV,
    "pack_weights_kernel": CONTROL, "pack_batch_kernel": CONTROL,
    "warp_kernel": WARP, "warp_vec8_kernel": WARP, "warp_vec_win_kernel": WARP, "corner_index_kernel": WARP,
    "warp_train_kernel": WARP_TRAIN, "warp_bwd_kernel": WARP_SCATTER,
    "agg_prepare_kernel": CONTROL, "agg_finalize_kernel": CONTROL, "agg_bwd_finalize_kernel": WARP_SCATTER,
    "wgrad_kernel": WGRAD, "wgrad_a1_kernel": WGRAD, "wgrad_a1_valu_kernel": WGRAD, "wgrad2d_kernel": WGRAD,
    "wgrad_lds_kernel": WGRAD, "wgrad_lds_batch_kernel": WGRAD, "slab_sum_kernel": WGRAD, "slab_sum_batch_kernel": WGRAD,
    "bn_reduce_kernel": BN, "bn_finalize_kernel": BN, "bn_relu_apply_kernel": BN, "bn_finalize_apply_kernel": BN,
    "bn_relu_bwd_kernel": BN,
    "prob_head_kernel": PROB, "prob_head_tiled_kernel": PROB, "prob_from_partials_kernel": PROB,
    "softmax_regress_bwd_kernel": PROB, "prob_conv_dgrad_kernel": PROB, "upsample2_bwd_kernel": PROB,
    "depth_regress_kernel": HEADS, "confidence_kernel": HEADS, "confidence_up2_kernel": HEADS, "range_affine_kernel": HEADS,
    "hypos_fit_kernel": HEADS, "hypos_from_fit_kernel": HEADS, "refine_head_kernel": HEADS, "fpn_compose_fwd_kernel": HEADS, "fpn_compose_bwd_kernel": HEADS,
    "consistency_fuse_kernel": FILTER,
    "consensus_fuse_kernel": FILTER, "consensus_scan_kernel": FILTER, "consensus_compact_kernel": FILTER,
    "pcd_reproj_kernel": FILTER, "pcd_cand_count_kernel": FILTER, "pcd_cand_place_kernel": FILTER, "pcd_select_kernel": FILTER, "pcd_select_big_kernel": FILTER, "pcd_bin_sum_kernel": FILTER, "pcd_bin_offsets_kernel": FILTER,
    "pcd_seg_init_kernel": FILTER, "pcd_seg_hook_kernel": FILTER, "pcd_seg_count_kernel": FILTER, "pcd_seg_apply_kernel": FILTER,
    "pcd_count_kernel": FILTER, "pcd_scan_kernel": FILTER, "pcd_compact_kernel": FILTER,
    "pts_bbox_kernel": POINT_EVAL, "pts_bbox_final_kernel": POINT_EVAL, "pts_morton_kernel": POINT_EVAL, "pts_sort_hist_kernel": POINT_EVAL,
    "pts_sort_scan_kernel": POINT_EVAL, "pts_sort_scatter_kernel": POINT_EVAL, "pts_gather_kernel": POINT_EVAL, "pts_leaf_kernel": POINT_EVAL,
    "pts_node_kernel": POINT_EVAL, "pts_nn_kernel": POINT_EVAL, "pts_rank_kernel": POINT_EVAL, "pts_radius_kernel": POINT_EVAL,
    "pts_reduce_init_kernel": POINT_EVAL, "pts_reduce_round_kernel": POINT_EVAL, "pts_reduce_step_kernel": POINT_EVAL,
    "pts_reduce_keep_kernel": POINT_EVAL, "pts_dtu_masks_kernel": POINT_EVAL,
    "masked_smooth_l1_reduce_kernel": CONTROL, "masked_smooth_l1_finalize_kernel": CONTROL, "masked_smooth_l1_bwd_kernel": CONTROL,
    "masked_smooth_l1_reduce_multi_kernel": CONTROL, "masked_smooth_l1_bwd_multi_kernel": CONTROL, "adam_step_kernel": CONTROL,
}

def function_name(rocprof_name):
    s = rocprof_name.strip()
    if s.startswith("void "):
        s = s[5:]
    s = s.replace("(anonymous namespace)::", "")
    head = re.split(r"[<(]", s, maxsplit=1)[0]
    return head.split("::")[-1].strip()


def family(rocprof_name):
    return KERNEL_FAMILY.get(function_name(rocprof_name))


def is_ours(rocprof_name):
    return function_name(rocprof_name) in KERNEL_FAMILY


def globals_in_sources(csrc_dir):
    import os
    names = {}
    for f in sorted(os.listdir(csrc_dir)):
        if not f.endswith(".hip"):
            continue
        text = open(os.path.join(csrc_dir, f)).read()
        for m in re.finditer(r"__global__\b[\s\S]*?\bvoid\s+([A-Za-z_][A-Za-z_0-9]*)\s*\(", text):
            names.setdefault(m.group(1), f)
    return names


def fetch_size_factor(rocprof_name):
    return 2.0
```

### mdf-net_amd/mdfnet_hip/ops.py

```python
import ctypes
import os
import threading

import torch

from . import check, lib

FEA_NHWC = 1
VOL_NCDHW, VOL_NDHWC = 0, 1

_prof = None


def profile_begin():
    global _prof
    _prof = []


def profile_end():
    global _prof
    recs, _prof = _prof, None
    torch.cuda.synchronize()
    return [(n, tag, e0.elapsed_time(e1), work) for n, tag, e0, e1, work in recs]


_counts = None


def count_begin():
    global _counts
    _counts = {}


def count_end():
    global _counts
    c, _counts = _counts, None
    return c


def _abi(name, args, tag="", work=None):
    fn = getattr(lib(), name)
    if _counts is not None:
        _counts[name] = _counts.get(name, 0) + 1
    if _prof is None:
        check(fn(*args), name)
        return
    e0, e1 = torch.cuda.Event(enable_timing=True), torch.cuda.Event(enable_timing=True)
    e0.record()
    check(fn(*args), name)
    e1.record()
    _prof.append((name, tag, e0, e1, dict(work or {}, kernel=lib().mdf_last_launch().decode())))


class _single_thread:

    def __enter__(self):
        self.n = torch.get_num_threads()
        if self.n > 1:
            torch.set_num_threads(1)

    def __exit__(self, *a):
        if self.n > 1:
            torch.set_num_threads(self.n)


_raw_stream = getattr(torch._C, "_cuda_getCurrentRawStream", None)


def _stream(t):
    if _raw_stream is not None:
        return ctypes.c_void_p(_raw_stream(t.device.index if t.device.index is not None else torch.cuda.current_device()))
    return ctypes.c_void_p(torch.cuda.current_stream(t.device).cuda_stream)


def _need_gpu(*ts):
    for t in ts:
        if t is not None and not t.is_cuda:
            raise RuntimeError("mdfnet_hip ops run on an MI355X only (got a CPU tensor); there is no CPU fallback")


def _f32c(t):
    return t if (t.dtype == torch.float32 and t.is_contiguous()) else t.float().contiguous()


def nhwc(t):
    return t.float().contiguous(memory_format=torch.channels_last)


_recorded = threading.local()


class recorded_host_values:
    def __init__(self, projs=None, fit_row=None, log_thresh=None, cams=None):
        self.v = {"projs": list(projs or []), "cams": list(cams or []), "fit_row": fit_row, "log_thresh": log_thresh or {}}

    def __enter__(self):
        _recorded.v = self.v
        return self

    def __exit__(self, *exc):
        _recorded.v = None


def recorded(kind, key=None):
    v = getattr(_recorded, "v", None)
    if v is None:
        return None
    if kind in ("projs", "cams"):
        return torch.as_tensor(v[kind].pop(0)).float().contiguous() if v[kind] else None
    if kind == "log_thresh":
        return v["log_thresh"].get(key)
    return None if v[kind] is None else torch.as_tensor(v[kind]).float().contiguous()


def relative_projections(ref_proj, src_projs):
    pinned = recorded("projs")
    if pinned is not None:
        return pinned
    ref = ref_proj.detach().to("cpu", torch.float32)
    with _single_thread():
        inv = torch.inverse(ref)
        rows = [torch.matmul(sp.detach().to("cpu", torch.float32), inv)[:, :3, :4].reshape(-1, 12) for sp in src_projs]
        return torch.stack(rows, 0).contiguous()


def _hypos_arg(hypos, h, w):
    per_pixel = int(hypos.shape[-1] != 1 or hypos.shape[-2] != 1)
    if per_pixel and (hypos.shape[-2] != h or hypos.shape[-1] != w):
        raise ValueError(f"depth_hypos {tuple(hypos.shape)} does not match feature size {(h, w)}")
    return _f32c(hypos), per_pixel


def homo_warp(src_fea, proj12, depth_hypos):
    _need_gpu(src_fea, proj12, depth_hypos)
    b, c, h, w = src_fea.shape
    d = depth_hypos.shape[1]
    fea = nhwc(src_fea)
    hyp, pp = _hypos_arg(depth_hypos, h, w)
    out = torch.empty((b, c, d, h, w), device=src_fea.device, dtype=torch.float32)
    _abi("mdf_homo_warp_fwd", (fea.data_ptr(), FEA_NHWC, _f32c(proj12).data_ptr(), hyp.data_ptr(), pp,
                                  out.data_ptr(), VOL_NCDHW, b, c, d, h, w, _stream(out),))
    return out


def warp_corner_indices(proj12, depth_hypos, h, w):
    _need_gpu(proj12, depth_hypos)
    b, d = depth_hypos.shape[:2]
    hyp, pp = _hypos_arg(depth_hypos, h, w)
    out = torch.empty((b, d, h, w, 2), device=proj12.device, dtype=torch.int32)
    _abi("mdf_warp_corner_indices", (_f32c(proj12).data_ptr(), hyp.data_ptr(), pp, out.data_ptr(), b, d, h, w,
                                        _stream(out),))
    return out


def _src_array(srcs):
    arr = (ctypes.c_void_p * len(srcs))(*[s.data_ptr() for s in srcs])
    return arr


def warp_aggregate_vec(features, proj, depth_hypos, w_params, ngroups, channels_last=True):
    _need_gpu(*features, proj, depth_hypos, w_params)
    feas = [nhwc(f) for f in features]
    b, c, h, w = feas[0].shape
    d = depth_hypos.shape[1]
    hyp, pp = _hypos_arg(depth_hypos, h, w)
    g = ngroups
    dev = feas[0].device
    if channels_last:
        mem = torch.empty((b, d, h, w, g), device=dev, dtype=torch.float32)
        cost = mem.permute(0, 4, 1, 2, 3)
    else:
        mem = cost = torch.empty((b, g, d, h, w), device=dev, dtype=torch.float32)
    srcs = feas[1:]
    _abi("mdf_warp_aggregate_vec_fwd", (feas[0].data_ptr(), _src_array(srcs), FEA_NHWC, _f32c(proj).data_ptr(),
                                           hyp.data_ptr(), pp, _f32c(w_params).data_ptr(), mem.data_ptr(),
                                           VOL_NDHWC if channels_last else VOL_NCDHW, b, c, g, d, h, w, len(srcs),
                                           _stream(mem),), tag=f"C{c}G{g}D{d} {w}x{h} V{len(feas)}",
         work={"bytes": 4.0 * b * (len(feas) * c * h * w + hyp.numel() / b + g * d * h * w),
               "bound": "hbm"})
    return cost


def warp_aggregate_var(features, proj, depth_hypos, channels_last=False):
    _need_gpu(*features, proj, depth_hypos)
    feas = [nhwc(f) for f in features]
    b, c, h, w = feas[0].shape
    d = depth_hypos.shape[1]
    hyp, pp = _hypos_arg(depth_hypos, h, w)
    dev = feas[0].device
    if channels_last:
        mem = torch.empty((b, d, h, w, c), device=dev, dtype=torch.float32)
        cost = mem.permute(0, 4, 1, 2, 3)
    else:
        mem = cost = torch.empty((b, c, d, h, w), device=dev, dtype=torch.float32)
    srcs = feas[1:]
    _abi("mdf_warp_aggregate_var_fwd", (feas[0].data_ptr(), _src_array(srcs), FEA_NHWC, _f32c(proj).data_ptr(),
                                           hyp.data_ptr(), pp, mem.data_ptr(),
                                           VOL_NDHWC if channels_last else VOL_NCDHW, b, c, d, h, w, len(srcs),
                                           _stream(mem),))
    return cost


def fold_view_weight(p, ngroups, prefix="depth_weight."):
    cw = p[prefix + "0.conv.weight"].reshape(ngroups).float()
    invstd = 1.0 / torch.sqrt(p[prefix + "0.bn.running_var"].float() + 1e-5)
    alpha = p[prefix + "0.bn.weight"].float() * invstd
    beta = p[prefix + "0.bn.bias"].float() - p[prefix + "0.bn.running_mean"].float() * alpha
    return torch.cat([cw, alpha.reshape(1), beta.reshape(1), p[prefix + "1.weight"].reshape(1).float(),
                      p[prefix + "1.bias"].reshape(1).float()]).contiguous()


def depth_regress(prob, depth_hypos):
    _need_gpu(prob, depth_hypos)
    b, d, h, w = prob.shape
    hyp, pp = _hypos_arg(depth_hypos, h, w)
    prob = _f32c(prob)
    out = torch.empty((b, h, w), device=prob.device, dtype=torch.float32)
    _abi("mdf_depth_regress_fwd", (prob.data_ptr(), hyp.data_ptr(), pp, out.data_ptr(), b, d, h, w, _stream(out),))
    return out


def confidence(prob, return_index=False):
    _need_gpu(prob)
    b, d, h, w = prob.shape
    prob = _f32c(prob)
    out = torch.empty((b, h, w), device=prob.device, dtype=torch.float32)
    idx = torch.empty((b, h, w), device=prob.device, dtype=torch.int64) if return_index else None
    _abi("mdf_confidence_fwd", (prob.data_ptr(), out.data_ptr(), idx.data_ptr() if return_index else None,
                                   b, d, h, w, _stream(out),))
    return (out, idx) if return_index else out


def confidence_up2(prob):
    _need_gpu(prob)
    b, d, h, w = prob.shape
    prob = _f32c(prob)
    out = torch.empty((b, 2 * h, 2 * w), device=prob.device, dtype=torch.float32)
    _abi("mdf_confidence_up2_fwd", (prob.data_ptr(), out.data_ptr(), b, d, h, w, _stream(out),))
    return out


def range_affine(x, lo, span, mode):
    _need_gpu(x, lo, span)
    x = _f32c(x)
    y = torch.empty_like(x)
    b = x.shape[0]
    lo_c, span_c = _f32c(lo), _f32c(span)
    _abi("mdf_range_affine_fwd", (x.data_ptr(), lo_c.data_ptr(), span_c.data_ptr(), mode, y.data_ptr(), b, x.numel() // b, _stream(y),))
    return y


_fit_row_cache = {}


def gauss1_fit_row(depth_hypos):
    pinned = recorded("fit_row")
    if pinned is not None:
        return pinned
    hyp = depth_hypos.detach().to("cpu", torch.float32)
    b, d = hyp.shape[:2]
    key = (b, d, hyp.numpy().tobytes())
    row = _fit_row_cache.get(key)
    if row is None:
        with _single_thread():
            rep = hyp.reshape(b, d, 1, 1).repeat(1, 1, 2, 2)
            x = torch.stack([rep ** 2, rep, torch.ones_like(rep)], dim=-1).permute(0, 2, 3, 1, 4)
            xt = x.transpose(-1, -2)
            row = torch.matmul(torch.inverse(torch.matmul(xt, x)), xt)[:, 0, 0, 0, :].contiguous()
        if len(_fit_row_cache) > 256:
            _fit_row_cache.clear()
        _fit_row_cache[key] = row
    return row


def hypos_fit(mode, prob, depth, depth_hypos, fit_row=None):
    _need_gpu(prob)
    b, d, h, w = prob.shape
    prob = _f32c(prob)
    hyp, pp = _hypos_arg(depth_hypos, h, w)
    out = torch.empty((b, h, w), device=prob.device, dtype=torch.float32)
    _abi("mdf_hypos_fit_fwd", (mode, prob.data_ptr(), None if depth is None else _f32c(depth).data_ptr(),
                                  hyp.data_ptr(), pp, None if fit_row is None else _f32c(fit_row).data_ptr(),
                                  out.data_ptr(), b, d, h, w, _stream(out),))
    return out


def hypos_from_fit(mode, s, depth, depth_range_f32, log_thresh, ndepths, upsample=True):
    _need_gpu(s, depth, depth_range_f32)
    b, h, w = s.shape
    ho, wo = (2 * h, 2 * w) if upsample else (h, w)
    out = torch.empty((b, ndepths, ho, wo), device=s.device, dtype=torch.float32)
    _abi("mdf_hypos_from_fit_fwd", (mode, _f32c(s).data_ptr(), _f32c(depth).data_ptr(),
                                       _f32c(depth_range_f32).data_ptr(), ctypes.c_float(log_thresh), out.data_ptr(),
                                       b, ndepths, h, w, int(upsample), _stream(out),))
    return out


def to_ndhwc(t):
    cl = t.permute(0, 2, 3, 4, 1)
    return cl if (cl.is_contiguous() and cl.dtype == torch.float32) else cl.float().contiguous()


def from_ndhwc(cl):
    return cl.permute(0, 4, 1, 2, 3)


def pack_conv3d_weight(w, transposed=False):
    _need_gpu(w)
    cin, cout = (w.shape[0], w.shape[1]) if transposed else (w.shape[1], w.shape[0])
    n = lib().mdf_conv3d_packed_size(cin, cout)
    out = torch.empty((n,), device=w.device, dtype=torch.float32)
    _abi("mdf_conv3d_pack_weights", (_f32c(w.detach()).data_ptr(), out.data_ptr(), cin, cout, int(transposed),
                                        _stream(out),))
    return out


def conv3d_ndhwc(x, wpack, cin, cout, stride=1, transposed=False, alpha=None, beta=None, relu=False, res=None):
    _need_gpu(x, wpack)
    b, d, h, w, c = x.shape
    assert c == cin and x.is_contiguous()
    if transposed:
        do, ho, wo = 2 * d, 2 * h, 2 * w
    elif stride == 2:
        do, ho, wo = (d - 1) // 2 + 1, (h - 1) // 2 + 1, (w - 1) // 2 + 1
    else:
        do, ho, wo = d, h, w
    y = torch.empty((b, do, ho, wo, cout), device=x.device, dtype=torch.float32)
    if res is not None:
        assert res.shape == y.shape and res.is_contiguous()
    _abi("mdf_conv3d_fwd", (x.data_ptr(), wpack.data_ptr(), None if alpha is None else alpha.data_ptr(),
                               None if beta is None else beta.data_ptr(), None if res is None else res.data_ptr(),
                               y.data_ptr(), b, d, h, w, cin, cout, stride, int(transposed), int(relu), _stream(y),),
         tag=f"{cin}->{cout} {'T' if transposed else 's%d' % stride} {d}x{h}x{w}",
         work={"flops": 2.0 * 27 * cin * cout * b * (d * h * w if transposed else do * ho * wo),
               "bytes": 4.0 * (x.numel() + y.numel() * (2 if res is not None else 1)), "bound": "mfma"})
    return y


STAT_SLICES = 16


def conv3d_train(x, wpack, cin, cout, stride, transposed, res, stat_mode, stat_out, stat_y=None, stat_aux=None):
    _need_gpu(x, wpack, stat_out)
    b, d, h, w, c = x.shape
    assert c == cin and x.is_contiguous()
    if transposed:
        do, ho, wo = 2 * d, 2 * h, 2 * w
    elif stride == 2:
        do, ho, wo = (d - 1) // 2 + 1, (h - 1) // 2 + 1, (w - 1) // 2 + 1
    else:
        do, ho, wo = d, h, w
    y = torch.empty((b, do, ho, wo, cout), device=x.device, dtype=torch.float32)
    if res is not None:
        assert res.shape == y.shape and res.is_contiguous()
    if stat_mode == 2:
        assert stat_y.shape == y.shape and stat_y.is_contiguous() and stat_aux.numel() == 4 * cout
    nslices = stat_out.numel() // (2 * cout)
    assert stat_out.numel() == nslices * 2 * cout and stat_out.dtype == torch.float64
    _abi("mdf_conv3d_train_fwd", (x.data_ptr(), wpack.data_ptr(), None if res is None else res.data_ptr(), y.data_ptr(), b, d, h, w, cin, cout,
                                  stride, int(transposed), stat_mode, None if stat_y is None else stat_y.data_ptr(),
                                  None if stat_aux is None else stat_aux.data_ptr(), stat_out.data_ptr(), nslices, _stream(y)),
         tag=f"{cin}->{cout} {'T' if transposed else 's%d' % stride} {d}x{h}x{w} +sums{stat_mode}",
         work={"flops": 2.0 * 27 * cin * cout * b * (d * h * w if transposed else do * ho * wo),
               "bytes": 4.0 * (x.numel() + y.numel() * (1 + (res is not None) + (stat_mode == 2))), "bound": "mfma"})
    return y


def conv2d_train(x, wpack, cin, cout, ksize, stride, planar_in, stat_mode, stat_out, ngroups, stat_y=None, stat_aux=None):
    _need_gpu(x, wpack, stat_out)
    if planar_in:
        b, c, h, w = x.shape
    else:
        b, h, w, c = x.shape
    assert c == cin and x.is_contiguous() and b % ngroups == 0
    pad = (ksize - 1) // 2
    ho, wo = (h + 2 * pad - ksize) // stride + 1, (w + 2 * pad - ksize) // stride + 1
    y = torch.empty((b, ho, wo, cout), device=x.device, dtype=torch.float32)
    if stat_mode == 2:
        assert stat_y.shape == y.shape and stat_y.is_contiguous() and stat_aux.numel() == ngroups * 4 * cout
    nslices = stat_out.numel() // (ngroups * 2 * cout)
    assert stat_out.numel() == nslices * ngroups * 2 * cout and stat_out.dtype == torch.float64
    _abi("mdf_conv2d_train_fwd", (x.data_ptr(), wpack.data_ptr(), y.data_ptr(), b, h, w, cin, cout, ksize, stride, int(planar_in), stat_mode,
                                  None if stat_y is None else stat_y.data_ptr(), None if stat_aux is None else stat_aux.data_ptr(),
                                  stat_out.data_ptr(), nslices, ngroups, _stream(y)),
         tag=f"{cin}->{cout} k{ksize}s{stride} {h}x{w}x{b} +sums{stat_mode}",
         work={"flops": 2.0 * ksize * ksize * cin * cout * b * ho * wo, "bytes": 4.0 * (x.numel() + y.numel() * (1 + (stat_mode == 2))),
               "bound": "mfma"})
    return y


def pack_prob_weight(weight):
    w = weight.detach().float()
    w2 = torch.zeros((4, w.shape[1], 3, 3), device=w.device, dtype=torch.float32)
    w2[:3] = w[0].permute(1, 0, 2, 3)
    return pack_conv2d_weight(w2)


PROB_FUSED = os.environ.get("MDF_PROB_FUSED", "1") != "0"
PROB_FUSED_MIN_TILES = int(os.environ.get("MDF_PROB_FUSED_MIN_TILES", "400"))


def prob_head(x, weight, depth_hypos=None, direct=False, wpack=None):
    _need_gpu(x, weight)
    b, d, h, w, c = x.shape
    prob = torch.empty((b, d, h, w), device=x.device, dtype=torch.float32)
    depth, hyp, pp = None, None, 0
    if depth_hypos is not None:
        hyp, pp = _hypos_arg(depth_hypos, h, w)
        depth = torch.empty((b, h, w), device=x.device, dtype=torch.float32)
    fused_lds = 2 * c * 398 * 4 + d * 1024
    if (not direct and c in (8, 16) and x.is_contiguous() and PROB_FUSED and fused_lds <= 160 * 1024
            and b * ((h + 3) // 4) * ((w + 63) // 64) >= PROB_FUSED_MIN_TILES):
        wp = pack_prob_weight(weight) if wpack is None else wpack
        _abi("mdf_prob_fused_fwd", (x.data_ptr(), wp.data_ptr(), None if hyp is None else hyp.data_ptr(), pp, prob.data_ptr(),
                                    None if depth is None else depth.data_ptr(), b, d, h, w, c, _stream(prob),),
             tag=f"{c}->1 {d}x{h}x{w}", work={"flops": 2.0 * 27 * c * b * d * h * w,
                                              "bytes": 4.0 * (x.numel() + prob.numel()), "bound": "hbm"})
        return prob if depth is None else (prob, depth)
    if not direct and c in (8, 16) and d <= 96 and x.is_contiguous():
        part = conv2d_nhwc(x.view(b * d, h, w, c), pack_prob_weight(weight) if wpack is None else wpack, c, 4, 3, 1,
                           useful_cout=3)
        _abi("mdf_prob_from_partials_fwd", (part.data_ptr(), None if hyp is None else hyp.data_ptr(), pp, prob.data_ptr(),
                                            None if depth is None else depth.data_ptr(), b, d, h, w, _stream(prob),),
             tag=f"partials->prob {d}x{h}x{w}", work={"bytes": 4.0 * (part.numel() + prob.numel()), "bound": "hbm"})
        return prob if depth is None else (prob, depth)
    _abi("mdf_prob_softmax_regress_fwd", (x.data_ptr(), _f32c(weight.detach()).data_ptr(),
                                             None if hyp is None else hyp.data_ptr(), pp, prob.data_ptr(),
                                             None if depth is None else depth.data_ptr(), b, d, h, w, c, _stream(prob),),
         tag=f"{c}->1 {d}x{h}x{w}", work={"flops": 2.0 * 27 * c * b * d * h * w,
                                          "bytes": 4.0 * (x.numel() + prob.numel()), "bound": "hbm"})
    return prob if depth is None else (prob, depth)


def refine_tail(x, w1pack, w2, lo=None, span=None):
    _need_gpu(x, w1pack, w2)
    b, h, w, c = x.shape
    assert c == 8 and x.is_contiguous() and tuple(w2.shape) == (1, 8, 3, 3)
    y = torch.empty((b, 2 * h, 2 * w), device=x.device, dtype=torch.float32)
    w2_c, lo_c, span_c = _f32c(w2.detach()), (None if lo is None else _f32c(lo)), (None if span is None else _f32c(span))
    _abi("mdf_refine_tail_fwd", (x.data_ptr(), w1pack.data_ptr(), w2_c.data_ptr(), None if lo_c is None else lo_c.data_ptr(),
                                 None if span_c is None else span_c.data_ptr(), y.data_ptr(), b, h, w, _stream(y),),
         tag=f"8->32->1 {h}x{w}x{b}", work={"flops": 2.0 * 72 * (32 + 4) * b * h * w, "bytes": 4.0 * (x.numel() + y.numel()), "bound": "mfma"})
    return y


def fold_bn(bn_weight, bn_bias, running_mean, running_var, eps=1e-5):
    invstd = 1.0 / torch.sqrt(running_var.float() + eps)
    alpha = (bn_weight.float() * invstd).contiguous()
    beta = (bn_bias.float() - running_mean.float() * alpha).contiguous()
    return alpha, beta


def pack_conv2d_weight(w):
    _need_gpu(w)
    cout, cin, k, _ = w.shape
    n = lib().mdf_conv_packed_size(cin, cout, k * k)
    out = torch.empty((n,), device=w.device, dtype=torch.float32)
    _abi("mdf_conv_pack_weights", (_f32c(w.detach()).data_ptr(), out.data_ptr(), cin, cout, k * k, _stream(out),))
    return out


def conv2d_nhwc(x, wpack, cin, cout, ksize, stride=1, alpha=None, beta=None, relu=False, res=None, res_scale=1.0,
                res_up=None, planar_in=False, useful_cout=None, pixel_shuffle2=False):
    _need_gpu(x, wpack)
    if planar_in:
        b, c, h, w = x.shape
    else:
        b, h, w, c = x.shape
    assert c == cin and x.is_contiguous()
    pad = (ksize - 1) // 2
    ho, wo = (h + 2 * pad - ksize) // stride + 1, (w + 2 * pad - ksize) // stride + 1
    y = torch.empty((b, 2 * ho, 2 * wo, cout // 4) if pixel_shuffle2 else (b, ho, wo, cout), device=x.device, dtype=torch.float32)
    _abi("mdf_conv2d_fwd", (x.data_ptr(), wpack.data_ptr(), None if alpha is None else alpha.data_ptr(),
                            None if beta is None else beta.data_ptr(), None if res is None else res.data_ptr(),
                            ctypes.c_float(res_scale), None if res_up is None else res_up.data_ptr(), y.data_ptr(),
                            b, h, w, cin, cout, ksize, stride, int(relu), int(planar_in), int(pixel_shuffle2), _stream(y),),
         tag=f"{cin}->{cout} k{ksize}s{stride} {h}x{w}x{b}",
         work={"flops": 2.0 * ksize * ksize * cin * (useful_cout or cout) * b * ho * wo, "bytes": 4.0 * (x.numel() + y.numel()),
               "bound": "mfma"})
    return y


def conv2d_pair_planar(x, w1pack, a1, b1, w2pack, a2, b2):
    _need_gpu(x, w1pack, w2pack)
    n, c, h, w = x.shape
    assert c == 3 and x.is_contiguous() and x.dtype == torch.float32
    y = torch.empty((n, h, w, 8), device=x.device, dtype=torch.float32)
    _abi("mdf_conv2d_pair_fwd", (x.data_ptr(), w1pack.data_ptr(), a1.data_ptr(), b1.data_ptr(), w2pack.data_ptr(), a2.data_ptr(), b2.data_ptr(),
                                 y.data_ptr(), n, h, w, _stream(y)), tag=f"3->8->8 k3 {h}x{w}x{n}",
         work={"flops": 2.0 * 9 * (3 * 8 + 8 * 8) * n * h * w, "bytes": 4.0 * (x.numel() + y.numel()), "bound": "mfma"})
    return y


def conv1x1_heads(x, heads, res_ups):
    _need_gpu(x)
    b, h, w, cin = x.shape
    assert x.is_contiguous() and all(hd[2] == cin for hd in heads)
    n = len(heads)
    ys = [torch.empty((b, h, w, hd[3]), device=x.device, dtype=torch.float32) for hd in heads]
    ptr = lambda t: None if t is None else t.data_ptr()
    wp = (ctypes.c_void_p * n)(*[hd[0].data_ptr() for hd in heads])
    bs = (ctypes.c_void_p * n)(*[ptr(hd[1]) for hd in heads])
    ru = (ctypes.c_void_p * n)(*[ptr(r) for r in res_ups])
    yo = (ctypes.c_void_p * n)(*[y.data_ptr() for y in ys])
    co = (ctypes.c_int * n)(*[hd[3] for hd in heads])
    for r, hd in zip(res_ups, heads):
        assert r is None or (tuple(r.shape) == (b, h // 2, w // 2, hd[3]) and r.is_contiguous())
    cout = sum(hd[3] for hd in heads)
    _abi("mdf_conv1x1_heads_fwd", (x.data_ptr(), n, wp, bs, ru, yo, co, b, h, w, cin, _stream(x)),
         tag=f"{cin}->{'/'.join(str(hd[3]) for hd in heads)} k1s1 {h}x{w}x{b}",
         work={"flops": 2.0 * cin * cout * b * h * w, "bytes": 4.0 * (x.numel() + sum(y.numel() for y in ys)), "bound": "mfma"})
    return ys


def refine_head(depth, lo, span, weight):
    _need_gpu(depth, weight)
    b, h, w = depth.shape
    assert tuple(weight.shape) == (8, 1, 3, 3)
    d, wt = _f32c(depth), _f32c(weight.detach())
    y = torch.empty((b, h, w, 8), device=depth.device, dtype=torch.float32)
    lo_c, span_c = (None if lo is None else _f32c(lo)), (None if span is None else _f32c(span))
    _abi("mdf_refine_head_fwd", (d.data_ptr(), None if lo_c is None else lo_c.data_ptr(), None if span_c is None else span_c.data_ptr(),
                                 wt.data_ptr(), y.data_ptr(), b, h, w, _stream(y)), tag=f"range + 1->8 k3 {h}x{w}x{b}",
         work={"bytes": 4.0 * (d.numel() + y.numel()), "bound": "hbm"})
    return y


def conv2d_res_pair(x, wa_pack, wb_pack, scale=0.1):
    _need_gpu(x, wa_pack, wb_pack)
    n, h, w, c = x.shape
    assert c == 8 and x.is_contiguous() and x.dtype == torch.float32
    y = torch.empty_like(x)
    _abi("mdf_conv2d_res_pair_fwd", (x.data_ptr(), wa_pack.data_ptr(), wb_pack.data_ptr(), ctypes.c_float(scale), y.data_ptr(), n, h, w, _stream(y)),
         tag=f"8->8->8 k3 res {h}x{w}x{n}", work={"flops": 2.0 * 9 * 2 * 8 * 8 * n * h * w, "bytes": 4.0 * (x.numel() + y.numel()), "bound": "mfma"})
    return y


def shuffle2_rows(weight):
    co = weight.shape[0]
    return weight.detach().reshape(co // 4, 4, *weight.shape[1:]).transpose(0, 1).reshape(weight.shape).contiguous()


def to_nhwc(t):
    cl = t.permute(0, 2, 3, 1)
    return cl if (cl.is_contiguous() and cl.dtype == torch.float32) else cl.float().contiguous()


def from_nhwc(cl):
    return cl.permute(0, 3, 1, 2)


def consistency_mats(k_ref, e_ref, src_ks, src_es):
    k_ref, e_ref = k_ref.detach().to("cpu", torch.float32), e_ref.detach().to("cpu", torch.float32)
    rows = []
    with _single_thread():
        kr_inv, er_inv = torch.inverse(k_ref), torch.inverse(e_ref)
        for k, e in zip(src_ks, src_es):
            k, e = k.detach().to("cpu", torch.float32), e.detach().to("cpu", torch.float32)
            rows.append(torch.cat([kr_inv.reshape(-1), torch.matmul(e, er_inv).reshape(-1), k.reshape(-1),
                                   torch.inverse(k).reshape(-1), torch.matmul(e_ref, torch.inverse(e)).reshape(-1),
                                   k_ref.reshape(-1)]))
    return torch.stack(rows).contiguous()


def consistency_fuse(depth_ref, conf, k_ref, e_ref, src_depths, src_ks, src_es, photo_threshold=0.8, nconditions=5,
                     thre1=4.0, thre2=1300.0, per_view=False):
    _need_gpu(depth_ref, conf, *src_depths)
    h, w = depth_ref.shape
    dev = depth_ref.device
    srcs = [_f32c(d) for d in src_depths]
    mats = consistency_mats(k_ref, e_ref, src_ks, src_es).to(dev, non_blocking=True)
    depth_avg = torch.empty((h, w), device=dev, dtype=torch.float32)
    masks = torch.empty((3, h, w), device=dev, dtype=torch.uint8)
    vm = torch.empty((len(srcs), h, w), device=dev, dtype=torch.int16) if per_view else None
    rep = torch.empty((len(srcs), h, w), device=dev, dtype=torch.float32) if per_view else None
    _abi("mdf_consistency_fuse_fwd", (_f32c(depth_ref).data_ptr(), _f32c(conf).data_ptr(), _src_array(srcs), mats.data_ptr(),
                                      len(srcs), h, w, ctypes.c_float(photo_threshold), int(nconditions),
                                      ctypes.c_float(thre1), ctypes.c_float(thre2), depth_avg.data_ptr(), masks.data_ptr(),
                                      None if vm is None else vm.data_ptr(), None if rep is None else rep.data_ptr(),
                                      _stream(depth_avg),),
         tag=f"{w}x{h} nsrc{len(srcs)}", work={"bytes": 4.0 * h * w * (len(srcs) + 3) + 3.0 * h * w, "bound": "hbm"})
    mb = masks.view(torch.bool)
    out = {"depth_avg": depth_avg, "photo_mask": mb[0], "geo_mask": mb[1], "final_mask": mb[2]}
    if per_view:
        bits = vm.to(torch.int32) & 0xFFFF
        out["view_masks"] = torch.stack([((bits >> i) & 1).bool() for i in range(9)], dim=1)
        out["rep"] = rep
    return out


CONSENSUS_CAM_STRIDE = 32


def consensus_cameras(K, E):
    import numpy as np
    K = np.asarray(K, dtype=np.float32).astype(np.float64)
    E = np.asarray(E, dtype=np.float32).astype(np.float64)
    n = K.shape[0]
    tab = np.zeros((n, CONSENSUS_CAM_STRIDE), dtype=np.float32)
    for v in range(n):
        P = (K[v] @ E[v][:3]).astype(np.float32)
        m_inv = np.linalg.inv(P[:, :3].astype(np.float64))
        tab[v, 0:12] = P.reshape(-1)
        tab[v, 12:21] = m_inv.astype(np.float32).reshape(-1)
        tab[v, 21:24] = (-(m_inv @ P[:, 3].astype(np.float64))).astype(np.float32)
    return tab, np.float32(K[0][0, 0])


def consensus_fuse(depths, images, K, E, disp_thresh, num_consistent):
    _need_gpu(depths, images)
    if depths.dim() != 3 or images.dim() != 4 or tuple(images.shape) != (*depths.shape, 3) or images.dtype != torch.uint8:
        raise ValueError(f"depths [N,H,W] fp32 and images [N,H,W,3] uint8 expected, got {tuple(depths.shape)} and "
                         f"{tuple(images.shape)} {images.dtype}")
    n, h, w = depths.shape
    dev = depths.device
    tab, f = consensus_cameras(K, E)
    cams = torch.from_numpy(tab).to(dev)
    colors = torch.nn.functional.pad(images, (0, 1)).contiguous()
    depths = _f32c(depths)
    ws = torch.empty(int(lib().mdf_consensus_fuse_workspace(n, h, w)), device=dev, dtype=torch.uint8)
    counts = torch.empty(n, device=dev, dtype=torch.int32)
    total = torch.empty(1, device=dev, dtype=torch.int64)
    _abi("mdf_consensus_fuse_fwd", (depths.data_ptr(), colors.data_ptr(), cams.data_ptr(), n, h, w, ctypes.c_float(float(f)),
                                    ctypes.c_float(disp_thresh), int(num_consistent), ws.data_ptr(), None, None, 0,
                                    counts.data_ptr(), total.data_ptr(), _stream(depths)),
         tag=f"{w}x{h} n{n}", work={"pairs": float(n) * (n - 1) * h * w, "bound": "valu"})
    m = int(total.item())
    xyz = torch.empty((m, 3), device=dev, dtype=torch.float32)
    rgb = torch.empty((m, 3), device=dev, dtype=torch.uint8)
    if m:
        _abi("mdf_consensus_compact", (ws.data_ptr(), n, h, w, xyz.data_ptr(), rgb.data_ptr(), m, _stream(depths)),
             tag=f"{w}x{h} n{n}", work={"bytes": 16.0 * n * h * w + 15.0 * m, "bound": "hbm"})
    return xyz, rgb, counts


PCD_CAM_STRIDE = 64
PCD_STEPS = ("prob", "vis1", "vis_fusion", "vis2", "ave", "vis3", "seg")
PCD_MAX_SOURCES = 64
PCD_PROB_THRESHOLD = 0.8


def pcd_cameras(K, E):
    import numpy as np
    K = np.asarray(K, dtype=np.float32)
    E = np.asarray(E, dtype=np.float32)
    tab = np.zeros((K.shape[0], PCD_CAM_STRIDE), dtype=np.float32)
    for v in range(K.shape[0]):
        k64, e64 = K[v].astype(np.float64), E[v].astype(np.float64)
        tab[v, 0:9] = K[v].ravel()
        tab[v, 9:18] = np.linalg.inv(k64).astype(np.float32).ravel()
        tab[v, 18:34] = E[v].ravel()
        tab[v, 34:50] = np.linalg.inv(e64).astype(np.float32).ravel()
        tab[v, 50:53] = (-(e64[:3, :3].T @ e64[:3, 3])).astype(np.float32)
    return tab


def pcd_sources(src_table, n, view):
    import numpy as np
    t = np.full((n, view), -1, dtype=np.int32)
    for i in range(n):
        s = [int(x) for x in list(src_table[i]) if int(x) >= 0][:view]
        if any(x >= n for x in s):
            raise ValueError(f"view {i}: source index out of range in {s}")
        t[i, :len(s)] = s
    return t


def pcd_steps(depths, masks, cams, srcs, need, first, last):
    n, h, w = depths.shape
    v = srcs.shape[1]
    dev = depths.device
    ws = torch.empty(int(lib().mdf_pcd_fuse_workspace(n, h, w, v)), device=dev, dtype=torch.uint8)
    counts = torch.empty(n, device=dev, dtype=torch.int32)
    total = torch.empty(1, device=dev, dtype=torch.int64)
    _abi("mdf_pcd_fuse_fwd", (depths.data_ptr(), masks.data_ptr(), cams.data_ptr(), srcs.data_ptr() if v else None, n, h, w, v,
                              int(need), int(first), int(last), ws.data_ptr(), counts.data_ptr(), total.data_ptr(),
                              _stream(depths)),
         tag=f"{w}x{h} n{n} v{v} steps{first}-{last}", work={"candidates": float(n) * (v + 1) * h * w, "bound": "valu"})
    return ws, counts, int(total.item())


def pcd_fuse(depths, probs, images, K, E, src_table, view=10, vthresh=4, normals=False, downsample=None, stages=None):
    import numpy as np
    if normals or downsample is not None:
        raise NotImplementedError("pcd_fuse: normal estimation and voxel downsampling are not implemented; "
                                  "call with normals=False, downsample=None")
    _need_gpu(depths, probs, images)
    if depths.dim() != 3 or tuple(probs.shape) != tuple(depths.shape) or tuple(images.shape) != (*depths.shape, 3) \
            or images.dtype != torch.uint8:
        raise ValueError(f"depths / probs [N,H,W] fp32 and images [N,H,W,3] uint8 expected, got {tuple(depths.shape)}, "
                         f"{tuple(probs.shape)} and {tuple(images.shape)} {images.dtype}")
    if not 0 <= view <= PCD_MAX_SOURCES:
        raise ValueError(f"view={view} out of range [0, {PCD_MAX_SOURCES}]")
    n, h, w = depths.shape
    dev = depths.device
    nsteps = len(PCD_STEPS) if stages is None else int(stages)
    if not 1 <= nsteps <= len(PCD_STEPS):
        raise ValueError(f"stages={stages} out of range [1, {len(PCD_STEPS)}]")
    cams = torch.from_numpy(pcd_cameras(K, E)).to(dev)
    srcs = torch.from_numpy(pcd_sources(src_table, n, view)).to(dev)
    need = int(np.ceil(np.float32(vthresh - 1.1)))
    masks = (probs > PCD_PROB_THRESHOLD).to(torch.uint8).contiguous()
    depths = (_f32c(depths) * masks).contiguous()
    ws, counts, m = pcd_steps(depths, masks, cams, srcs, need, 1, nsteps - 1) if nsteps > 1 else \
        pcd_steps(depths, masks, cams, srcs, need, 1, 0)
    out = {"depths": depths, "masks": masks.bool(), "counts": counts}
    if stages is not None:
        return out
    xyz = torch.empty((m, 3), device=dev, dtype=torch.float32)
    rgb = torch.empty((m, 3), device=dev, dtype=torch.uint8)
    dirs = torch.empty((m, 3), device=dev, dtype=torch.float32)
    if m:
        images = images.contiguous()
        _abi("mdf_pcd_compact", (depths.data_ptr(), masks.data_ptr(), images.data_ptr(), cams.data_ptr(), n, h, w,
                                 view, ws.data_ptr(), xyz.data_ptr(), rgb.data_ptr(), dirs.data_ptr(), m, _stream(depths)),
             tag=f"{w}x{h} n{n}", work={"bytes": 5.0 * n * h * w + 27.0 * m, "bound": "hbm"})
    out.update(xyz=xyz, rgb=rgb, dirs=dirs)
    return out


DTU_MAX_DIST_CP = 60.0
DTU_OUTLIER = 20.0
DTU_MARGIN = 10
REDUCE_ROUNDS_PER_CALL = 32


class PointIndex:

    def __init__(self, buf, n, device):
        self.buf, self.n, self.device = buf, int(n), device

    @property
    def nbytes(self):
        return int(self.buf.numel())


def _pts64(pts, device=None):
    if not torch.is_tensor(pts):
        import numpy as np
        pts = torch.from_numpy(np.ascontiguousarray(np.asarray(pts, dtype=np.float64)))
    if not pts.is_cuda:
        if device is None:
            raise RuntimeError("mdfnet_hip ops run on an MI355X only (got a CPU tensor); there is no CPU fallback")
        pts = pts.to(device)
    pts = pts.to(torch.float64).reshape(-1, 3).contiguous() if pts.numel() else pts.new_zeros((0, 3), dtype=torch.float64)
    return pts


def point_index(pts):
    _need_gpu(pts)
    pts = _pts64(pts)
    n = pts.shape[0]
    nbytes = int(lib().mdf_pts_index_workspace(n))
    if nbytes <= 0 and n:
        raise ValueError(f"point_index: {n} points are too many")
    buf = torch.empty(max(nbytes, 16), device=pts.device, dtype=torch.uint8)
    _abi("mdf_pts_index_build", (pts.data_ptr() if n else None, n, buf.data_ptr(), buf.numel(), _stream(buf)), tag=f"n{n}",
         work={"points": float(n), "bound": "hbm"})
    return PointIndex(buf, n, pts.device)


def _host_doubles(vals, k):
    import numpy as np
    a = np.ascontiguousarray(np.asarray(vals, dtype=np.float64).reshape(-1))
    if a.size != k:
        raise ValueError(f"{k} values expected, got {a.size}")
    return (ctypes.c_double * k)(*a.tolist())


def nn_distance(index, queries, bb=None, cap=DTU_MAX_DIST_CP, return_visits=False):
    if not isinstance(index, PointIndex):
        raise TypeError("nn_distance: index must come from point_index()")
    if isinstance(queries, PointIndex):
        m, qidx, qpts, qbytes = queries.n, queries.buf.data_ptr(), None, queries.nbytes
    else:
        _need_gpu(queries)
        q = _pts64(queries)
        m, qidx, qpts, qbytes = q.shape[0], None, q.data_ptr(), 0
    dev = index.device
    dist = torch.empty(m, device=dev, dtype=torch.float64)
    visits = torch.empty(m, device=dev, dtype=torch.int32) if return_visits else None
    bbh = _host_doubles(bb, 6) if bb is not None else None
    if m:
        _abi("mdf_pts_nn_dist", (index.buf.data_ptr(), index.n, index.nbytes, qidx, qpts, m, qbytes, bbh, float(cap), dist.data_ptr(),
                                 visits.data_ptr() if visits is not None else None, _stream(dist)),
             tag=f"n{index.n} m{m}", work={"queries": float(m), "bound": "valu"})
    return (dist, visits) if return_visits else dist


def reduce_points(pts, dst, order, index=None, stats=None):
    import numpy as np
    _need_gpu(pts)
    pts = _pts64(pts)
    n = pts.shape[0]
    dev = pts.device
    if not (float(dst) > 0 and np.isfinite(float(dst))):
        raise ValueError(f"dst={dst} must be finite and > 0")
    order = torch.as_tensor(np.asarray(order) if not torch.is_tensor(order) else order).to(dev, torch.int64).reshape(-1)
    if order.numel() != n:
        raise ValueError(f"order has {order.numel()} entries for {n} points")
    rank = torch.empty(n, device=dev, dtype=torch.int32)
    if n:
        if bool(((order < 0) | (order >= n)).any()) or int(torch.bincount(order, minlength=n).max()) != 1:
            raise ValueError("order must be a permutation of 0..n-1")
        rank[order] = torch.arange(n, device=dev, dtype=torch.int32)
    index = index if index is not None else point_index(pts)
    if index.n != n:
        raise ValueError(f"index over {index.n} points for {n} points")
    ws = torch.empty(max(int(lib().mdf_pts_reduce_workspace(n)), 16), device=dev, dtype=torch.uint8)
    edges = torch.zeros(1, device=dev, dtype=torch.int64)
    args = (index.buf.data_ptr(), n, index.nbytes, rank.data_ptr() if n else None, ctypes.c_double(float(dst)), ws.data_ptr(), ws.numel())
    _abi("mdf_pts_reduce_count", args + (edges.data_ptr(), _stream(ws)), tag=f"n{n}", work={"points": float(n), "bound": "valu"})
    ne = int(edges.item())
    csr = torch.empty(max(ne, 1), device=dev, dtype=torch.int32)
    keep = torch.empty(max(n, 1), device=dev, dtype=torch.uint8)
    state = torch.zeros(3, device=dev, dtype=torch.int32)
    resume = 0
    while True:
        _abi("mdf_pts_reduce", args + (csr.data_ptr(), ne, resume, REDUCE_ROUNDS_PER_CALL, keep.data_ptr(), state.data_ptr(),
                                       _stream(ws)), tag=f"n{n} e{ne}", work={"edges": float(ne), "bound": "latency"})
        rounds, undecided, overflow = (int(x) for x in state.tolist())
        if overflow:
            raise RuntimeError(f"reduce_points: the neighbour lists did not fit ({ne} edges)")
        if undecided == 0:
            break
        resume = 1
    if stats is not None:
        stats.update(edges=ne, rounds=rounds)
    return keep[:n].bool(), rounds


def dtu_masks(qdata, obs_mask, bb, res, qstl, plane):
    import numpy as np
    _need_gpu(qdata, qstl)
    q, s = _pts64(qdata), _pts64(qstl)
    dev = q.device
    if torch.is_tensor(obs_mask):
        dims = tuple(obs_mask.shape)
        om = obs_mask.to(dev).permute(*reversed(range(obs_mask.dim()))).contiguous().reshape(-1).to(torch.uint8)
    else:
        a = np.asarray(obs_mask)
        dims = a.shape
        om = torch.from_numpy(np.ascontiguousarray(a.reshape(-1, order="F")).astype(np.uint8)).to(dev)
    dims = tuple(dims) + (1,) * (3 - len(dims))
    if len(dims) != 3:
        raise ValueError(f"ObsMask must be 3-D, got shape {dims}")
    n, m = q.shape[0], s.shape[0]
    in_mask = torch.empty(max(n, 1), device=dev, dtype=torch.uint8)
    above = torch.empty(max(m, 1), device=dev, dtype=torch.uint8)
    om = om if om.numel() else torch.zeros(1, device=dev, dtype=torch.uint8)
    _abi("mdf_dtu_masks", (q.data_ptr(), n, om.data_ptr(), int(dims[0]), int(dims[1]), int(dims[2]), _host_doubles(bb, 6),
                           ctypes.c_double(float(res)), in_mask.data_ptr(), s.data_ptr(), m, _host_doubles(plane, 4), above.data_ptr(),
                           _stream(q)), tag=f"n{n} m{m}", work={"points": float(n + m), "bound": "hbm"})
    return in_mask[:n].bool(), above[:m].bool()


def dtu_stats(d):
    import numpy as np
    d = np.asarray(d, dtype=np.float64).reshape(-1)
    if d.size == 0:
        return 0, float("nan"), float("nan"), float("nan")
    return int(d.size), float(np.mean(d)), float(np.var(d, ddof=1)) if d.size > 1 else 0.0, float(np.median(d))


def dtu_scan_stats(ev, max_dist=DTU_OUTLIER):
    import numpy as np
    dd = np.asarray(ev["Ddata"], dtype=np.float64).reshape(-1)
    ds = np.asarray(ev["Dstl"], dtype=np.float64).reshape(-1)
    dd = dd[np.asarray(ev["DataInMask"], dtype=bool).reshape(-1)]
    ds = ds[np.asarray(ev["StlAbovePlane"], dtype=bool).reshape(-1)]
    nd, md, vd, medd = dtu_stats(dd[dd < max_dist])
    ns, ms, vs, meds = dtu_stats(ds[ds < max_dist])
    return {"nData": nd, "MeanData": md, "VarData": vd, "MedData": medd, "nStl": ns, "MeanStl": ms, "VarStl": vs, "MedStl": meds}


def dtu_eval_scan(qdata, qstl, obs_mask, bb, res, plane, dst=0.2, seed=0, max_dist=DTU_OUTLIER, device=None):
    import numpy as np
    dev = torch.device(device) if device is not None else torch.device("cuda", torch.cuda.current_device())
    q = _pts64(qdata, dev)
    s = _pts64(qstl, dev)
    n = q.shape[0]
    order = np.random.RandomState(seed).permutation(n)
    stats = {}
    keep, _ = reduce_points(q, dst, order, stats=stats)
    qr = q[keep].contiguous()
    bb = np.asarray(bb, dtype=np.float64).reshape(2, 3)
    stl_index = point_index(s)
    data_index = point_index(qr)
    ddata = nn_distance(stl_index, data_index, bb=bb, cap=DTU_MAX_DIST_CP)
    dstl = nn_distance(data_index, stl_index, bb=bb, cap=DTU_MAX_DIST_CP)
    in_mask, above = dtu_masks(qr, obs_mask, bb, res, s, plane)
    ev = {"Qdata": qr.cpu().numpy().T.copy(), "Ddata": ddata.cpu().numpy(), "Qstl": s.cpu().numpy().T.copy(), "Dstl": dstl.cpu().numpy(),
          "DataInMask": in_mask.cpu().numpy(), "StlAbovePlane": above.cpu().numpy(),
          "GroundPlane": np.asarray(plane, dtype=np.float64).reshape(4, 1), "dst": float(dst), "Margin": DTU_MARGIN,
          "Rounds": stats["rounds"], "Edges": stats["edges"]}
    ev.update(dtu_scan_stats(ev, max_dist))
    return ev
```

### mdf-net_amd/net/core.py

```python
import torch

from mdfnet_hip import controlplane, hostmirror, layers, ops


import contextlib
import os as _os

_STAGE_STREAMS = bool(int(_os.environ.get("MDF_TRAIN_STAGE_STREAMS", "1")))
_SIDE = {}


def _stage_streams(device, n):
    key = (device.index if device.index is not None else torch.cuda.current_device(), n)
    if key not in _SIDE:
        _SIDE[key] = [torch.cuda.Stream(device) for _ in range(n)]
    return _SIDE[key]


@contextlib.contextmanager
def _on_stage_stream(side, stage, main, feats):
    if not side:
        yield
        return
    st = side[stage]
    st.wait_stream(main)
    for f in feats:
        base = getattr(f, "_mdf_parent", None)
        (base[0] if base is not None else f).record_stream(st)
    with torch.cuda.stream(st):
        yield
    main.wait_stream(st)


def _cut_features(feats, cuts):
    parents = [getattr(f, "_mdf_parent", None) for f in feats]
    pairs = []
    if all(p is not None and p[0] is parents[0][0] and p[1] == i and p[2] == len(feats) for i, p in enumerate(parents)):
        y = parents[0][0]
        yc = y.detach().requires_grad_(True)
        b = y.shape[0] // len(feats)
        out = [yc[g * b:(g + 1) * b] for g in range(len(feats))]
        for g, t in enumerate(out):
            t._mdf_parent = (yc, g, len(feats))
        pairs.append((y, yc))
    else:
        out = [f.detach().requires_grad_(True) for f in feats]
        pairs.extend(zip(feats, out))
    cuts.feat.append(pairs)
    return out


class CoreNet(torch.nn.Module):
    def __init__(self, Backbone, Depth_hypos, scale, Homoaggre, Regular, Regress, Refine):
        super().__init__()
        self.Backbone, self.Depth_hypos, self.scale = Backbone, Depth_hypos, scale
        self.Homoaggre, self.Regular, self.Refine = Homoaggre, Regular, Refine
        self.Depth_regress, self.Confidence_regress = Regress
        print("{} parameters: {}".format(self._get_name(), sum(p.data.nelement() for p in self.parameters())))

    def forward(self, origin_imgs, extrinsics, intrinsics, depth_range, feature_cache=None, view_keys=None):
        with layers.model_mode(self.training):
            plan = None
            if origin_imgs.is_cuda:
                hostmirror.ensure((extrinsics, intrinsics, depth_range))
                plan = controlplane.prepare(self, intrinsics, extrinsics, depth_range)
            with controlplane.active(plan):
                return self._forward(origin_imgs, extrinsics, intrinsics, depth_range, feature_cache, view_keys)

    def _pyramids(self, imgs, feature_cache, view_keys):
        nb, nv = imgs.shape[:2]
        if feature_cache is not None and view_keys is not None and nb == 1 and not self.training:
            if hasattr(feature_cache, "pin"):
                feature_cache.pin(view_keys)
            missing = [v for v in range(nv) if view_keys[v] not in feature_cache]
            if missing:
                f = self.Backbone(imgs[0, missing])
                ev = torch.cuda.Event()
                ev.record()
                for j, v in enumerate(missing):
                    feature_cache[view_keys[v]] = (tuple(lv[j:j + 1] for lv in f), ev)
            cur = torch.cuda.current_stream(imgs.device)
            out = []
            for v in range(nv):
                pyr, ev = feature_cache[view_keys[v]]
                cur.wait_event(ev)
                for t in pyr:
                    t.record_stream(cur)
                out.append(pyr)
            return out
        if self.training and imgs.is_cuda and hasattr(self.Backbone, "forward_views") and layers.hip_train(self.Backbone, imgs):
            return self.Backbone.forward_views(imgs)
        if getattr(self.Backbone, "batch_views", False) and not self.training:
            f = self.Backbone(imgs.reshape(nb * nv, *imgs.shape[2:]))
            return [tuple(lv.reshape(nb, nv, *lv.shape[1:])[:, v] for lv in f) for v in range(nv)]
        return [self.Backbone(v) for v in torch.unbind(imgs, 1)]

    def _forward(self, origin_imgs, extrinsics, intrinsics, depth_range, feature_cache=None, view_keys=None):
        if not self.training and not origin_imgs.is_cuda:
            raise RuntimeError("CoreNet inference runs on hand-written MI355X kernels only: move the model and inputs to a "
                               "GPU (there is no CPU fallback; model.train() on a GPU runs the hand-written training kernels)")
        if origin_imgs.is_cuda:
            hostmirror.ensure((extrinsics, intrinsics, depth_range))
        if self.training and origin_imgs.is_cuda and layers.hip_train(self, origin_imgs):
            from mdfnet_hip import train_ops
            with torch.no_grad():
                train_ops.prepack(self)
        pyramids = self._pyramids(origin_imgs.float(), feature_cache, view_keys)
        depth = hypos = prob = None
        depths = []
        side = cuts = None
        if self.training and origin_imgs.is_cuda and torch.is_grad_enabled() and layers.hip_train(self, origin_imgs):
            cuts = layers.active_cuts()
            if cuts is not None or (_STAGE_STREAMS and not torch.cuda.is_current_stream_capturing()):
                side = _stage_streams(origin_imgs.device, len(self.Regular))
                main = torch.cuda.current_stream(origin_imgs.device)
                if cuts is not None:
                    cuts.streams = side
        for stage, (make_hypos, aggregate, regular) in enumerate(zip(self.Depth_hypos, self.Homoaggre, self.Regular)):
            feats = [p[stage] for p in pyramids]
            if cuts is not None:
                feats = _cut_features(feats, cuts)
            ref_proj, src_projs = self.scale(intrinsics, extrinsics, stage)
            with _on_stage_stream(side, stage, main if side else None, feats):
                hypos = make_hypos(depth, depth_range, prob, hypos, upsample=True)
                cost = aggregate(feats, ref_proj, src_projs, hypos)
                if ((not self.training or cost.is_cuda) and getattr(regular, "fused_regress", False)
                        and getattr(self.Depth_regress, "mdf_builtin", False)):
                    prob, depth = regular(cost, hypos)
                else:
                    prob = regular(cost)
                    depth = self.Depth_regress(prob, hypos)
            if side:
                for t in (hypos, prob, depth):
                    t.record_stream(main)
                    if stage + 1 < len(side):
                        t.record_stream(side[stage + 1])
            if cuts is not None:
                cut = depth.detach().requires_grad_(True)
                cuts.depth.append((depth, cut))
                depth = cut
            depths.append(depth)
        depth = self.Refine(depth, depth_range)
        if cuts is not None and depth.requires_grad:
            cut = depth.detach().requires_grad_(True)
            cuts.refine = (depth, cut)
            depth = cut
        depths.append(depth)
        if self.training:
            return {"depth": depths}
        if getattr(self.Confidence_regress, "mdf_builtin", False) and prob.is_cuda:
            conf = ops.confidence_up2(prob.detach())
        else:
            conf = self.Confidence_regress(prob)
            conf = torch.nn.functional.interpolate(conf.unsqueeze(1), scale_factor=2, mode="nearest").squeeze(1)
        return {"depth": depth, "confidence": conf}
```

### mdf-net_amd/net/unit/backbone.py

```python
from typing import Tuple

import torch
import torch.nn as nn
import torch.nn.functional as F

from mdfnet_hip import layers, ops
from .base import ConvBNReLU


import os as _os
_HEADS = bool(int(_os.environ.get("MDF_FPN_HEADS_FUSED", "1")))
_PAIR = bool(int(_os.environ.get("MDF_CONV_PAIR", "1")))


def _stage(cin, cout, first_k, first_s):
    return nn.Sequential(ConvBNReLU(cin, cout, first_k, first_s, (first_k - 1) // 2), ConvBNReLU(cout, cout, 3, 1, 1),
                         ConvBNReLU(cout, cout, 3, 1, 1))


class FPN_4Scales(nn.Module):
    batch_views = True

    def __init__(self, out_chs: Tuple = (8, 16, 32, 64)) -> None:
        super().__init__()
        c0, c1, c2, c3 = out_chs
        self.conv01 = nn.Sequential(ConvBNReLU(3, c0, 3, 1, 1), ConvBNReLU(c0, c0, 3, 1, 1))
        self.conv12 = _stage(c0, c1, 5, 2)
        self.conv23 = _stage(c1, c2, 5, 2)
        self.conv34 = _stage(c2, c3, 5, 2)
        self.lat2 = nn.Conv2d(c1, c3, 1, bias=True)
        self.lat3 = nn.Conv2d(c2, c3, 1, bias=True)
        self.out2 = nn.Conv2d(c3, c1, 1, bias=False)
        self.out3 = nn.Conv2d(c3, c2, 1, bias=False)
        self.out4 = nn.Conv2d(c3, c3, 1, bias=False)

    def _composed_heads(self):
        mods = (self.out2, self.out3, self.out4, self.lat2, self.lat3)
        tensors = [t for m in mods for t in (m.weight, m.bias) if t is not None]

        def build():
            def mat(m):
                return m.weight.detach().double().reshape(m.out_channels, m.in_channels)
            o2, o3, l2, l3 = mat(self.out2), mat(self.out3), mat(self.lat2), mat(self.lat3)
            b2, b3 = self.lat2.bias.detach().double(), self.lat3.bias.detach().double()

            def pack(w, bias=None):
                w4 = w.float().reshape(w.shape[0], w.shape[1], 1, 1).contiguous()
                return ops.pack_conv2d_weight(w4), (None if bias is None else bias.float().contiguous()), w.shape[1], w.shape[0]
            return {"y4": pack(mat(self.out4)), "a4": pack(o3), "y3": pack(o3 @ l3, o3 @ b3),
                    "c4": pack(o2), "c3": pack(o2 @ l3, o2 @ b3), "y2": pack(o2 @ l2, o2 @ b2)}
        return layers.cache_of(self.out2).get(tensors, build)

    def _hip_forward(self, x):
        def seq(blocks, t):
            for blk in blocks:
                t = layers.conv2d_layer(blk.conv, blk.bn, t, relu=True)
            return t

        def head(h, t, res_up=None):
            wp, bias, cin, cout = h
            return ops.conv2d_nhwc(t, wp, cin, cout, 1, 1, None, bias, False, None, 1.0, res_up)
        with torch.no_grad():
            first, second = self.conv01[0], self.conv01[1]
            xin = x.float().contiguous()
            if _PAIR and first.conv.in_channels == 3 and first.conv.out_channels == 8 and second.conv.out_channels == 8 and len(self.conv01) == 2:
                t1 = layers.conv2d_pair(first, second, xin)
            else:
                t1 = layers.conv2d_layer(first.conv, first.bn, xin, relu=True, planar_in=True)
                t1 = seq(self.conv01[1:], t1)
            t2 = seq(self.conv12, t1)
            t3 = seq(self.conv23, t2)
            t4 = seq(self.conv34, t3)
            hd = self._composed_heads()
            if _HEADS and (hd["y4"][2], hd["y4"][3], hd["a4"][3], hd["c4"][3], hd["y3"][2], hd["y3"][3], hd["c3"][2], hd["c3"][3]) == (64, 64, 32, 16, 32, 32, 32, 16) \
                    and tuple(t3.shape[1:3]) == (2 * t4.shape[1], 2 * t4.shape[2]):
                y4, a4, c4 = ops.conv1x1_heads(t4, [hd["y4"], hd["a4"], hd["c4"]], [None, None, None])
                y3, c3 = ops.conv1x1_heads(t3, [hd["y3"], hd["c3"]], [a4, c4])
            else:
                y4 = head(hd["y4"], t4)
                y3 = head(hd["y3"], t3, res_up=head(hd["a4"], t4))
                c3 = head(hd["c3"], t3, res_up=head(hd["c4"], t4))
            y2 = head(hd["y2"], t2, res_up=c3)
        return ops.from_nhwc(y4), ops.from_nhwc(y3), ops.from_nhwc(y2)

    def _heads(self, t2, t3, t4):
        if layers.hip_train(self, t2, t3, t4):
            from mdfnet_hip import train_ops
            return train_ops.fpn_heads_train(self, t2, t3, t4)
        up3 = F.interpolate(t4, scale_factor=2.0, mode="bilinear", align_corners=False) + self.lat3(t3)
        up2 = F.interpolate(up3, scale_factor=2.0, mode="bilinear", align_corners=False) + self.lat2(t2)
        return self.out4(t4), self.out3(up3), self.out2(up2)

    def forward_views(self, imgs):
        from mdfnet_hip import train_ops
        b, v = imgs.shape[:2]
        x = imgs.transpose(0, 1).reshape(v * b, *imgs.shape[2:])
        ys = self._heads(*train_ops.trunk_train(self, x, groups=v))
        out = []
        for g in range(v):
            trip = tuple(y[g * b:(g + 1) * b] for y in ys)
            for t, y in zip(trip, ys):
                t._mdf_parent = (y, g, v)
            out.append(trip)
        return out

    def forward(self, x: torch.Tensor):
        if layers.hip_eval(self, x):
            return self._hip_forward(x)
        if layers.hip_train(self, x):
            from mdfnet_hip import train_ops
            return self._heads(*train_ops.trunk_train(self, x, groups=1))
        t2 = self.conv12(self.conv01(x))
        t3 = self.conv23(t2)
        t4 = self.conv34(t3)
        up3 = F.interpolate(t4, scale_factor=2.0, mode="bilinear", align_corners=False) + self.lat3(t3)
        up2 = F.interpolate(up3, scale_factor=2.0, mode="bilinear", align_corners=False) + self.lat2(t2)
        return self.out4(t4), self.out3(up3), self.out2(up2)
```

### mdf-net_amd/net/unit/homoaggregate.py

```python
import torch
import torch.nn as nn

from mdfnet_hip import controlplane, hostmirror, layers, ops
from .base import ConvBNReLU3D


def _projections(ref_proj, src_projs, device):
    ready = controlplane.projections(ref_proj)
    if ready is not None and ready.shape[0] == len(src_projs):
        return ready
    host = ops.relative_projections(hostmirror.get(ref_proj), [hostmirror.get(s) for s in src_projs])
    return host.to(device, non_blocking=True)


class VectorAggregate(nn.Module):

    def __init__(self, ngroups: int = 8):
        super().__init__()
        self.ngroups = ngroups
        self.depth_weight = nn.Sequential(ConvBNReLU3D(ngroups, 1, 1, 1, 0), nn.Conv3d(1, 1, 1, 1, 0), nn.Sigmoid())

    def _params(self):
        sd = {k: v for k, v in self.depth_weight.state_dict(keep_vars=True).items()}
        return layers.cache_of(self).get(list(sd.values()), lambda: ops.fold_view_weight(sd, self.ngroups, prefix=""))

    def forward(self, features, ref_proj, src_projs, depth_hypos):
        if layers.hip_train(self, *features, depth_hypos):
            from mdfnet_hip import train_ops
            proj = _projections(ref_proj, src_projs, features[0].device)
            return train_ops.aggregate_train(self, list(features), proj, depth_hypos)
        if not layers.use_hip(self, *features, depth_hypos):
            return layers.stock().vector_aggregate(self.depth_weight, self.ngroups, features, ref_proj, src_projs, depth_hypos)
        with torch.no_grad():
            proj = _projections(ref_proj, src_projs, features[0].device)
            return ops.warp_aggregate_vec(list(features), proj, depth_hypos, self._params(), self.ngroups)


def homo_aggregate_by_variance(features, ref_proj, src_projs, depth_hypos):
    if not layers.use_hip(None, *features, depth_hypos):
        return layers.stock().variance_aggregate(features, ref_proj, src_projs, depth_hypos)
    with torch.no_grad():
        proj = _projections(ref_proj, src_projs, features[0].device)
        return ops.warp_aggregate_var(list(features), proj, depth_hypos)
```

Before: 278.7 views/s.

## Fold pair-difference into FPN heads and aggregate from half-width difference maps

Composes the FPN output head weights into pairwise row differences, so the backbone emits maps with half the channels (one per group, a difference of channel pairs). A new warp-aggregate kernel gathers only these difference maps and rebuilds the group similarity through a sigmoid-based form. This is meant to halve the gather bandwidth and the head output size in cost-volume construction. It relies on the similarity being expressible through per-pair differences with group size 2, and adds support for head outputs that are not a multiple of 16 channels.

```diff
diff --git a/include/mdfnet_hip.h b/include/mdfnet_hip.h
--- a/include/mdfnet_hip.h
+++ b/include/mdfnet_hip.h
@@ -38,6 +38,11 @@
                                const float* proj, const float* hypos, int hypos_per_pixel,
                                const float* w_params, float* cost, int cost_layout, int B, int C, int G,
                                int D, int h, int w, int n_src, void* stream);
+
+int mdf_warp_aggregate_pairdiff_fwd(const float* ref_diff, const float* const* src_diffs, int fea_layout,
+                                    const float* proj, const float* hypos, int hypos_per_pixel,
+                                    const float* w_params, float* cost, int cost_layout, int B, int G, int D,
+                                    int h, int w, int n_src, void* stream);
 
 int mdf_warp_aggregate_var_fwd(const float* ref_fea, const float* const* src_feas, int fea_layout,
                                const float* proj, const float* hypos, int hypos_per_pixel, float* cost,
diff --git a/mdf-net_amd/csrc/conv1x1.hip b/mdf-net_amd/csrc/conv1x1.hip
--- a/mdf-net_amd/csrc/conv1x1.hip
+++ b/mdf-net_amd/csrc/conv1x1.hip
@@ -35,7 +35,7 @@
 
 template <int CIN, int COUT>
 __global__ __launch_bounds__(256) void conv1x1_kernel(const P1 p) {
-  constexpr int NCH = CIN / 16, NT = COUT / 16;
+  constexpr int NCH = CIN / 16, NT = (COUT + 15) / 16;
   constexpr int U = (8 / NCH) < 1 ? 1 : 8 / NCH;
   const int lane = threadIdx.x & 63, q = lane >> 4, n16 = lane & 15;
   const int wave_g = blockIdx.x * 4 + (threadIdx.x >> 6), n_waves = gridDim.x * 4;
@@ -54,8 +54,8 @@
 #pragma unroll
     for (int k = 0; k < 4; ++k) {
       const int c = nt * 16 + 4 * q + k;
-      al[nt][k] = p.alpha ? p.alpha[c] : 1.f;
-      be[nt][k] = p.beta ? p.beta[c] : 0.f;
+      al[nt][k] = (p.alpha && c < COUT) ? p.alpha[c] : 1.f;
+      be[nt][k] = (p.beta && c < COUT) ? p.beta[c] : 0.f;
     }
 
   for (int run = wave_g; run < p.n_runs; run += n_waves) {
@@ -90,6 +90,7 @@
 #pragma unroll
       for (int nt = 0; nt < NT; ++nt) {
         const int c0 = nt * 16 + 4 * q;
+        if (COUT % 16 != 0 && c0 >= COUT) continue;
         float o[4];
 #pragma unroll
         for (int k = 0; k < 4; ++k) {
@@ -140,7 +141,7 @@
 template <int CIN, int C0, int C1, int C2, int U>
 __global__ __launch_bounds__(256) void conv1x1_heads_kernel(const P1M p) {
   constexpr int NCH = CIN / 16;
-  constexpr int N0 = C0 / 16, N1 = C1 / 16, N2 = C2 / 16, NT = N0 + N1 + N2;
+  constexpr int N0 = (C0 + 15) / 16, N1 = (C1 + 15) / 16, N2 = (C2 + 15) / 16, NT = N0 + N1 + N2;
   const int lane = threadIdx.x & 63, q = lane >> 4, n16 = lane & 15;
   const int wave_g = blockIdx.x * 4 + (threadIdx.x >> 6), n_waves = gridDim.x * 4;
   auto head_of = [](int nt) { return nt < N0 ? 0 : (nt < N0 + N1 ? 1 : 2); };
@@ -153,7 +154,7 @@
   float be[NT][4];
 #pragma unroll
   for (int nt = 0; nt < NT; ++nt) {
-    const int h = head_of(nt), lt = nt - first_of(h), nth = cout_of(h) / 16;
+    const int h = head_of(nt), lt = nt - first_of(h), nth = (cout_of(h) + 15) / 16;
 #pragma unroll
     for (int ch = 0; ch < NCH; ++ch) {
       if constexpr (WLDS) {
@@ -165,7 +166,7 @@
       }
     }
 #pragma unroll
-    for (int k = 0; k < 4; ++k) be[nt][k] = p.beta[h] ? p.beta[h][lt * 16 + 4 * q + k] : 0.f;
+    for (int k = 0; k < 4; ++k) be[nt][k] = (p.beta[h] && lt * 16 + 4 * q + k < cout_of(h)) ? p.beta[h][lt * 16 + 4 * q + k] : 0.f;
   }
   if constexpr (WLDS) __syncthreads();
 
@@ -218,6 +219,7 @@
 #pragma unroll
       for (int nt = 0; nt < NT; ++nt) {
         const int h = head_of(nt), co = cout_of(h), c0 = (nt - first_of(h)) * 16 + 4 * q;
+        if (co % 16 != 0 && c0 >= co) continue;
         float o[4];
 #pragma unroll
         for (int k = 0; k < 4; ++k) o[k] = acc[nt][k] * 1.0f + be[nt][k];
@@ -277,6 +279,7 @@
   p.res_scale = res_scale; p.relu = relu; p.Ho = H; p.Wo = W; p.npx = (long long)B * H * W;
   if (p.npx >= (1ll << 31) - 256) return MDF_EUNSUPPORTED;
   C1_CASE(16, 16) C1_CASE(16, 32) C1_CASE(16, 64) C1_CASE(32, 16) C1_CASE(32, 32) C1_CASE(32, 64)
+  C1_CASE(16, 8)
   return MDF_EUNSUPPORTED;
 }
 
@@ -299,5 +302,7 @@
   hipStream_t st = (hipStream_t)stream;
   if (Cin == 64 && n_heads == 3 && couts[0] == 64 && couts[1] == 32 && couts[2] == 16) return launch_heads<64, 64, 32, 16, 1>(p, st);
   if (Cin == 32 && n_heads == 2 && couts[0] == 32 && couts[1] == 16) return launch_heads<32, 32, 16, 0, 1>(p, st);
-  return mdf::fail(MDF_EUNSUPPORTED, "conv1x1 heads: Cin=%d with %d heads is not built (64 -> 64/32/16, 32 -> 32/16)", Cin, n_heads);
-}
+  if (Cin == 64 && n_heads == 3 && couts[0] == 32 && couts[1] == 16 && couts[2] == 8) return launch_heads<64, 32, 16, 8, 1>(p, st);
+  if (Cin == 32 && n_heads == 2 && couts[0] == 16 && couts[1] == 8) return launch_heads<32, 16, 8, 0, 1>(p, st);
+  return mdf::fail(MDF_EUNSUPPORTED, "conv1x1 heads: Cin=%d with %d heads is not built (64 -> 64/32/16, 32 -> 32/16, 64 -> 32/16/8, 32 -> 16/8)", Cin, n_heads);
+}
diff --git a/mdf-net_amd/csrc/warp_aggregate.hip b/mdf-net_amd/csrc/warp_aggregate.hip
--- a/mdf-net_amd/csrc/warp_aggregate.hip
+++ b/mdf-net_amd/csrc/warp_aggregate.hip
@@ -336,6 +336,172 @@
   if (lds > 64 * 1024) return MDF_EUNSUPPORTED;
   hipLaunchKernelGGL((warp_vec8_kernel<C>), dim3(p.nblk_x, p.B), dim3(kThreads), lds, st, p);
   return mdf::check_launch("warp_vec8_kernel");
+}
+
+template <int G, int GPL, bool FIXED>
+__global__ __launch_bounds__(kThreads) void warp_pairdiff_kernel(const Params p) {
+  static_assert(GPL == 4 || GPL == 8, "groups per lane");
+  static_assert(G % GPL == 0, "a pixel is a whole number of lanes");
+  constexpr int LPP = G / GPL;
+  constexpr int PPB = kThreads / LPP;
+  constexpr int NQ = GPL / 4;
+  extern __shared__ __attribute__((aligned(16))) char smem[];
+  TapEntry* tab = reinterpret_cast<TapEntry*>(smem);
+  const int hw = p.g.h * p.g.w;
+  const int b = blockIdx.y;
+  const PixTile<PPB> pt((int)mdf::xcd_remap(blockIdx.x, p.nblk_x), p.g.w);
+  const int tid = threadIdx.x;
+  const int pl = tid / LPP, sub = tid % LPP;
+  bool live;
+  const int pix = pt.pix(pl, p.g.w, p.g.h, live);
+
+  float rd[GPL], r1[GPL], cw[GPL];
+#pragma unroll
+  for (int j = 0; j < NQ; ++j) {
+    const float4 rv = *reinterpret_cast<const float4*>(p.ref + ((size_t)b * hw + pix) * G + GPL * sub + 4 * j);
+    const float d4[4] = {rv.x, rv.y, rv.z, rv.w};
+#pragma unroll
+    for (int k = 0; k < 4; ++k) {
+      const float p0 = __builtin_amdgcn_rcpf(1.0f + __builtin_amdgcn_exp2f(d4[k] * kLog2e));
+      const float p1 = 1.0f - p0;
+      rd[4 * j + k] = p0 - p1; r1[4 * j + k] = p1;
+      cw[4 * j + k] = p.wpar[GPL * sub + 4 * j + k];
+    }
+  }
+  const float alpha = p.wpar[G], beta = p.wpar[G + 1], w2 = p.wpar[G + 2], b2 = p.wpar[G + 3];
+  const size_t map_stride = (size_t)hw * G;
+  const unsigned lane_b = 4u * GPL * (unsigned)sub;
+
+  const int npair = PPB * p.n_src;
+  const bool few = (npair <= kThreads) && (kThreads % npair) == 0;
+  const bool two = (npair == 2 * kThreads);
+  const int pa_ngrp = few ? kThreads / npair : 1, pa_grp = few ? tid / npair : 0;
+  PixelRay ray[2];
+  int pa_pl[2], pa_v[2], pa_pix[2];
+  if constexpr (FIXED) {
+#pragma unroll
+    for (int k = 0; k < 2; ++k) {
+      const int pair = (few ? tid % npair : tid) + k * kThreads;
+      pa_pl[k] = pair % PPB; pa_v[k] = min(pair / PPB, p.n_src - 1);
+      bool pa_live;
+      pa_pix[k] = pt.pix(pa_pl[k], p.g.w, p.g.h, pa_live);
+      const int yy = pa_pix[k] / p.g.w, xx = pa_pix[k] - yy * p.g.w;
+      ray[k] = warp_ray(p.proj + ((size_t)pa_v[k] * p.B + b) * 12, (float)xx, (float)yy);
+    }
+  }
+
+  for (int d0 = 0; d0 < p.D; d0 += p.dchunk) {
+    const int nd = min(p.dchunk, p.D - d0);
+    if constexpr (FIXED) {
+#pragma unroll
+      for (int k = 0; k < 2; ++k) {
+        if (k == 1 && !two) break;
+        for (int ed = pa_grp; ed < nd; ed += pa_ngrp) {
+          const int d = d0 + ed;
+          const float dep = p.hypos_per_pixel ? p.hypos[((size_t)b * p.D + d) * hw + pa_pix[k]] : p.hypos[(size_t)b * p.D + d];
+          float ix, iy;
+          warp_position_ray(ray[k], dep, p.g, ix, iy);
+          TapEntry t;
+          make_taps(ix, iy, p.g, G, t);
+          tab[(ed * p.n_src + pa_v[k]) * PPB + pa_pl[k]] = t;
+        }
+      }
+    } else {
+      const int nent = nd * p.n_src * PPB;
+      for (int e = tid; e < nent; e += kThreads) {
+        const int epl = e % PPB;
+        const int ev = (e / PPB) % p.n_src;
+        const int ed = e / (PPB * p.n_src);
+        bool elive;
+        const int epix = pt.pix(epl, p.g.w, p.g.h, elive);
+        const int yy = epix / p.g.w, xx = epix - yy * p.g.w;
+        const float* m = p.proj + ((size_t)ev * p.B + b) * 12;
+        const int d = d0 + ed;
+        const float dep = p.hypos_per_pixel ? p.hypos[((size_t)b * p.D + d) * hw + epix] : p.hypos[(size_t)b * p.D + d];
+        float ix, iy;
+        warp_position(m, (float)xx, (float)yy, dep, p.g, ix, iy);
+        TapEntry t;
+        make_taps(ix, iy, p.g, G, t);
+        tab[e] = t;
+      }
+    }
+    __syncthreads();
+    for (int dd = 0; dd < nd; ++dd) {
+      float acc[GPL];
+#pragma unroll
+      for (int k = 0; k < GPL; ++k) acc[k] = 0.f;
+      float wsum = 0.f;
+      for (int v = 0; v < p.n_src; ++v) {
+        const TapEntry t = tab[(dd * p.n_src + v) * PPB + pl];
+        const char* sb = reinterpret_cast<const char*>(p.src[v] + (size_t)b * map_stride);
+        float sim[GPL];
+        float part = 0.f;
+#pragma unroll
+        for (int j = 0; j < NQ; ++j) {
+          const unsigned lb = lane_b + 16u * j;
+          const float4 nw = *reinterpret_cast<const float4*>(sb + ((unsigned)t.off[0] * 4u + lb));
+          const float4 ne = *reinterpret_cast<const float4*>(sb + ((unsigned)t.off[1] * 4u + lb));
+          const float4 sw = *reinterpret_cast<const float4*>(sb + ((unsigned)t.off[2] * 4u + lb));
+          const float4 se = *reinterpret_cast<const float4*>(sb + ((unsigned)t.off[3] * 4u + lb));
+          float dv[4];
+          dv[0] = __fmaf_rn(se.x, t.wt[3], __fmaf_rn(sw.x, t.wt[2], __fmaf_rn(ne.x, t.wt[1], __fmul_rn(nw.x, t.wt[0]))));
+          dv[1] = __fmaf_rn(se.y, t.wt[3], __fmaf_rn(sw.y, t.wt[2], __fmaf_rn(ne.y, t.wt[1], __fmul_rn(nw.y, t.wt[0]))));
+          dv[2] = __fmaf_rn(se.z, t.wt[3], __fmaf_rn(sw.z, t.wt[2], __fmaf_rn(ne.z, t.wt[1], __fmul_rn(nw.z, t.wt[0]))));
+          dv[3] = __fmaf_rn(se.w, t.wt[3], __fmaf_rn(sw.w, t.wt[2], __fmaf_rn(ne.w, t.wt[1], __fmul_rn(nw.w, t.wt[0]))));
+          float q[2];
+#pragma unroll
+          for (int h2 = 0; h2 < 2; ++h2) {
+            const int g0 = 4 * j + 2 * h2;
+            sim[g0] = __fmaf_rn(__builtin_amdgcn_rcpf(1.0f + __builtin_amdgcn_exp2f(dv[2 * h2] * kLog2e)), rd[g0], r1[g0]);
+            sim[g0 + 1] = __fmaf_rn(__builtin_amdgcn_rcpf(1.0f + __builtin_amdgcn_exp2f(dv[2 * h2 + 1] * kLog2e)), rd[g0 + 1], r1[g0 + 1]);
+            q[h2] = __fmaf_rn(cw[g0], sim[g0], cw[g0 + 1] * sim[g0 + 1]);
+          }
+          part = (j == 0) ? (q[0] + q[1]) : (part + (q[0] + q[1]));
+        }
+        float z = part;
+        if constexpr (LPP > 1) z = pixel_sum<LPP>(part);
+        const float u = __fmaf_rn(fmaxf(__fmaf_rn(z, alpha, beta), 0.0f), w2, b2);
+        const float wv = __builtin_amdgcn_rcpf(1.0f + __builtin_amdgcn_exp2f(-u * kLog2e));
+        wsum += wv;
+#pragma unroll
+        for (int k = 0; k < GPL; ++k) acc[k] += wv * sim[k];
+      }
+      if (!live) continue;
+      const size_t vox = ((size_t)b * p.D + d0 + dd) * hw + pix;
+      if (p.out_ndhwc) {
+#pragma unroll
+        for (int j = 0; j < NQ; ++j) {
+          typedef float f4v __attribute__((ext_vector_type(4)));
+          f4v ov = {acc[4 * j] / wsum, acc[4 * j + 1] / wsum, acc[4 * j + 2] / wsum, acc[4 * j + 3] / wsum};
+          __builtin_nontemporal_store(ov, reinterpret_cast<f4v*>(p.out + vox * G + GPL * sub + 4 * j));
+        }
+      } else {
+        const size_t cs = (size_t)p.D * hw;
+        float* o = p.out + ((size_t)b * G * p.D + d0 + dd) * hw + pix;
+#pragma unroll
+        for (int k = 0; k < GPL; ++k) o[(size_t)(GPL * sub + k) * cs] = acc[k] / wsum;
+      }
+    }
+    __syncthreads();
+  }
+}
+
+template <int G, int GPL>
+int launch_pairdiff(Params& p, hipStream_t st) {
+  constexpr int ppb = kThreads / (G / GPL);
+  p.nblk_x = PixTile<ppb>::blocks(p.g.w, p.g.h);
+  int dch = MDF_VEC8_TAB / (p.n_src * ppb);
+  if (dch < 1) dch = 1;
+  if (dch > p.D) dch = p.D;
+  p.dchunk = dch;
+  const size_t lds = (size_t)dch * p.n_src * ppb * sizeof(TapEntry);
+  if (lds > 64 * 1024) return MDF_EUNSUPPORTED;
+  const int npair = ppb * p.n_src;
+  if ((npair <= kThreads && kThreads % npair == 0) || npair == 2 * kThreads)
+    hipLaunchKernelGGL((warp_pairdiff_kernel<G, GPL, true>), dim3(p.nblk_x, p.B), dim3(kThreads), lds, st, p);
+  else
+    hipLaunchKernelGGL((warp_pairdiff_kernel<G, GPL, false>), dim3(p.nblk_x, p.B), dim3(kThreads), lds, st, p);
+  return mdf::check_launch("warp_pairdiff_kernel");
 }
 
 struct WinDesc {
@@ -623,6 +789,42 @@
   return launch<kVec>(p, C, (hipStream_t)stream);
 }
 
+extern "C" int mdf_warp_aggregate_pairdiff_fwd(const float* ref_diff, const float* const* src_diffs, int fea_layout,
+                                               const float* proj, const float* hypos, int hypos_per_pixel,
+                                               const float* w_params, float* cost, int cost_layout, int B, int G, int D,
+                                               int h, int w, int n_src, void* stream) {
+  MDF_REQUIRE(ref_diff && src_diffs && proj && hypos && w_params && cost, "null pointer argument");
+  MDF_REQUIRE(B > 0 && D > 0 && h > 1 && w > 1, "bad shape B=%d D=%d h=%d w=%d", B, D, h, w);
+  MDF_REQUIRE((long long)h * w * G < (1ll << 30), "feature map too large for 32-bit byte offsets");
+  MDF_REQUIRE(n_src >= 1 && n_src <= MDF_MAX_SRC_VIEWS, "n_src=%d out of range [1,%d]", n_src, MDF_MAX_SRC_VIEWS);
+  if (fea_layout != MDF_FEA_NHWC)
+    return mdf::fail(MDF_EUNSUPPORTED, "feature layout %d not supported (kernels gather NHWC taps)", fea_layout);
+  if (G != 8 && G != 16 && G != 32)
+    return mdf::fail(MDF_EUNSUPPORTED, "G=%d not supported (pair-difference maps are built for 8, 16, 32 groups)", G);
+  Params p{};
+  p.ref = ref_diff;
+  for (int v = 0; v < n_src; ++v) {
+    MDF_REQUIRE(src_diffs[v], "src_diffs[%d] is null", v);
+    p.src[v] = src_diffs[v];
+  }
+  p.proj = proj; p.hypos = hypos; p.wpar = w_params; p.out = cost;
+  p.g = make_geom(h, w);
+  p.B = B; p.D = D; p.n_src = n_src; p.hypos_per_pixel = hypos_per_pixel; p.out_ndhwc = (cost_layout == MDF_VOL_NDHWC);
+  hipStream_t st = (hipStream_t)stream;
+  int gpl = 4;
+  if (const char* e = getenv("MDF_PAIRDIFF_GPL")) { if (atoi(e) == 4 || atoi(e) == 8) gpl = atoi(e); }
+  if (gpl == 8) {
+    int rc = MDF_EUNSUPPORTED;
+    if (G == 32) rc = launch_pairdiff<32, 8>(p, st);
+    else if (G == 16) rc = launch_pairdiff<16, 8>(p, st);
+    else rc = launch_pairdiff<8, 8>(p, st);
+    if (rc != MDF_EUNSUPPORTED) return rc;
+  }
+  if (G == 32) return launch_pairdiff<32, 4>(p, st);
+  if (G == 16) return launch_pairdiff<16, 4>(p, st);
+  return launch_pairdiff<8, 4>(p, st);
+}
+
 extern "C" int mdf_warp_aggregate_var_fwd(const float* ref_fea, const float* const* src_feas, int fea_layout,
                                           const float* proj, const float* hypos, int hypos_per_pixel, float* cost,
                                           int cost_layout, int B, int C, int D, int h, int w, int n_src, void* stream) {
diff --git a/mdf-net_amd/mdfnet_hip/__init__.py b/mdf-net_amd/mdfnet_hip/__init__.py
--- a/mdf-net_amd/mdfnet_hip/__init__.py
+++ b/mdf-net_amd/mdfnet_hip/__init__.py
@@ -24,6 +24,8 @@
     "mdf_warp_corner_indices": (c_int, [c_fp, c_fp, c_int, c_fp] + [c_int] * 4 + [c_fp]),
     "mdf_warp_aggregate_vec_fwd": (c_int, [c_fp, ctypes.POINTER(c_fp), c_int, c_fp, c_fp, c_int, c_fp, c_fp, c_int]
                                    + [c_int] * 7 + [c_fp]),
+    "mdf_warp_aggregate_pairdiff_fwd": (c_int, [c_fp, ctypes.POINTER(c_fp), c_int, c_fp, c_fp, c_int, c_fp, c_fp, c_int]
+                                        + [c_int] * 6 + [c_fp]),
     "mdf_warp_aggregate_var_fwd": (c_int, [c_fp, ctypes.POINTER(c_fp), c_int, c_fp, c_fp, c_int, c_fp, c_int]
                                    + [c_int] * 6 + [c_fp]),
     "mdf_conv3d_fwd": (c_int, [c_fp] * 6 + [c_int] * 9 + [c_fp]),
diff --git a/mdf-net_amd/mdfnet_hip/kernel_families.py b/mdf-net_amd/mdfnet_hip/kernel_families.py
--- a/mdf-net_amd/mdfnet_hip/kernel_families.py
+++ b/mdf-net_amd/mdfnet_hip/kernel_families.py
@@ -17,7 +17,7 @@
     "conv1x1_kernel": MFMA_CONV, "conv1x1_heads_kernel": MFMA_CONV, "refine_tail_kernel": MFMA_CONV, "prob_fused_kernel": MFMA_CONV, "res_pair_kernel": MFMA_CONV,
     "wino3d_kernel": MFMA_CONV, "wino2d_kernel": MFMA_CONV,
     "pack_weights_kernel": CONTROL, "pack_batch_kernel": CONTROL,
-    "warp_kernel": WARP, "warp_vec8_kernel": WARP, "warp_vec_win_kernel": WARP, "corner_index_kernel": WARP,
+    "warp_kernel": WARP, "warp_vec8_kernel": WARP, "warp_pairdiff_kernel": WARP, "warp_vec_win_kernel": WARP, "corner_index_kernel": WARP,
     "warp_train_kernel": WARP_TRAIN, "warp_bwd_kernel": WARP_SCATTER,
     "agg_prepare_kernel": CONTROL, "agg_finalize_kernel": CONTROL, "agg_bwd_finalize_kernel": WARP_SCATTER,
     "wgrad_kernel": WGRAD, "wgrad_a1_kernel": WGRAD, "wgrad_a1_valu_kernel": WGRAD, "wgrad2d_kernel": WGRAD,
diff --git a/mdf-net_amd/mdfnet_hip/ops.py b/mdf-net_amd/mdfnet_hip/ops.py
--- a/mdf-net_amd/mdfnet_hip/ops.py
+++ b/mdf-net_amd/mdfnet_hip/ops.py
@@ -177,6 +177,30 @@
                                            VOL_NDHWC if channels_last else VOL_NCDHW, b, c, g, d, h, w, len(srcs),
                                            _stream(mem),), tag=f"C{c}G{g}D{d} {w}x{h} V{len(feas)}",
          work={"bytes": 4.0 * b * (len(feas) * c * h * w + hyp.numel() / b + g * d * h * w),
+               "bound": "hbm"})
+    return cost
+
+
+def warp_aggregate_pairdiff(diffs, proj, depth_hypos, w_params, channels_last=True):
+    _need_gpu(*diffs, proj, depth_hypos, w_params)
+    feas = [nhwc(f) for f in diffs]
+    b, g, h, w = feas[0].shape
+    if w_params.numel() != g + 4:
+        raise ValueError(f"w_params has {w_params.numel()} entries, expected G + 4 = {g + 4}: are these pair-difference maps?")
+    d = depth_hypos.shape[1]
+    hyp, pp = _hypos_arg(depth_hypos, h, w)
+    dev = feas[0].device
+    if channels_last:
+        mem = torch.empty((b, d, h, w, g), device=dev, dtype=torch.float32)
+        cost = mem.permute(0, 4, 1, 2, 3)
+    else:
+        mem = cost = torch.empty((b, g, d, h, w), device=dev, dtype=torch.float32)
+    srcs = feas[1:]
+    _abi("mdf_warp_aggregate_pairdiff_fwd", (feas[0].data_ptr(), _src_array(srcs), FEA_NHWC, _f32c(proj).data_ptr(),
+                                             hyp.data_ptr(), pp, _f32c(w_params).data_ptr(), mem.data_ptr(),
+                                             VOL_NDHWC if channels_last else VOL_NCDHW, b, g, d, h, w, len(srcs),
+                                             _stream(mem),), tag=f"G{g}D{d} {w}x{h} V{len(feas)}",
+         work={"bytes": 4.0 * b * (len(feas) * g * h * w + hyp.numel() / b + g * d * h * w),
                "bound": "hbm"})
     return cost
 
diff --git a/mdf-net_amd/net/core.py b/mdf-net_amd/net/core.py
--- a/mdf-net_amd/net/core.py
+++ b/mdf-net_amd/net/core.py
@@ -50,6 +50,13 @@
     return out
 
 
+def _cached_form(cache, key):
+    if key not in cache:
+        return None
+    entry = dict.get(cache, key) if isinstance(cache, dict) else cache[key]
+    return bool(entry[2]) if len(entry) > 2 else False
+
+
 class CoreNet(torch.nn.Module):
     def __init__(self, Backbone, Depth_hypos, scale, Homoaggre, Regular, Regress, Refine):
         super().__init__()
@@ -67,22 +74,35 @@
             with controlplane.active(plan):
                 return self._forward(origin_imgs, extrinsics, intrinsics, depth_range, feature_cache, view_keys)
 
-    def _pyramids(self, imgs, feature_cache, view_keys):
+    def _pair_diff_route(self, imgs):
+        from .unit import backbone as _bb
+        from .unit.homoaggregate import VectorAggregate
+        bb = self.Backbone
+        if not _bb._PAIR_DIFF or self.training or not imgs.is_cuda or type(bb) is not _bb.FPN_4Scales:
+            return False
+        chans = (bb.out4.out_channels, bb.out3.out_channels, bb.out2.out_channels)
+        if chans != (64, 32, 16) or (bb.out4.in_channels, bb.lat3.in_channels, bb.lat2.in_channels) != (64, 32, 16):
+            return False
+        slots = list(self.Homoaggre)
+        return len(slots) == 3 and all(type(a) is VectorAggregate and 2 * a.ngroups == c for a, c in zip(slots, chans))
+
+    def _pyramids(self, imgs, feature_cache, view_keys, pair_diff=False):
         nb, nv = imgs.shape[:2]
+        backbone = (lambda x: self.Backbone(x, pair_diff=True)) if pair_diff else self.Backbone
         if feature_cache is not None and view_keys is not None and nb == 1 and not self.training:
             if hasattr(feature_cache, "pin"):
                 feature_cache.pin(view_keys)
-            missing = [v for v in range(nv) if view_keys[v] not in feature_cache]
+            missing = [v for v in range(nv) if _cached_form(feature_cache, view_keys[v]) is not pair_diff]
             if missing:
-                f = self.Backbone(imgs[0, missing])
+                f = backbone(imgs[0, missing])
                 ev = torch.cuda.Event()
                 ev.record()
                 for j, v in enumerate(missing):
-                    feature_cache[view_keys[v]] = (tuple(lv[j:j + 1] for lv in f), ev)
+                    feature_cache[view_keys[v]] = (tuple(lv[j:j + 1] for lv in f), ev, pair_diff)
             cur = torch.cuda.current_stream(imgs.device)
             out = []
             for v in range(nv):
-                pyr, ev = feature_cache[view_keys[v]]
+                pyr, ev = feature_cache[view_keys[v]][:2]
                 cur.wait_event(ev)
                 for t in pyr:
                     t.record_stream(cur)
@@ -91,9 +111,9 @@
         if self.training and imgs.is_cuda and hasattr(self.Backbone, "forward_views") and layers.hip_train(self.Backbone, imgs):
             return self.Backbone.forward_views(imgs)
         if getattr(self.Backbone, "batch_views", False) and not self.training:
-            f = self.Backbone(imgs.reshape(nb * nv, *imgs.shape[2:]))
+            f = backbone(imgs.reshape(nb * nv, *imgs.shape[2:]))
             return [tuple(lv.reshape(nb, nv, *lv.shape[1:])[:, v] for lv in f) for v in range(nv)]
-        return [self.Backbone(v) for v in torch.unbind(imgs, 1)]
+        return [backbone(v) for v in torch.unbind(imgs, 1)]
 
     def _forward(self, origin_imgs, extrinsics, intrinsics, depth_range, feature_cache=None, view_keys=None):
         if not self.training and not origin_imgs.is_cuda:
@@ -105,7 +125,8 @@
             from mdfnet_hip import train_ops
             with torch.no_grad():
                 train_ops.prepack(self)
-        pyramids = self._pyramids(origin_imgs.float(), feature_cache, view_keys)
+        pair_diff = self._pair_diff_route(origin_imgs)
+        pyramids = self._pyramids(origin_imgs.float(), feature_cache, view_keys, pair_diff)
         depth = hypos = prob = None
         depths = []
         side = cuts = None
@@ -123,7 +144,7 @@
             ref_proj, src_projs = self.scale(intrinsics, extrinsics, stage)
             with _on_stage_stream(side, stage, main if side else None, feats):
                 hypos = make_hypos(depth, depth_range, prob, hypos, upsample=True)
-                cost = aggregate(feats, ref_proj, src_projs, hypos)
+                cost = aggregate(feats, ref_proj, src_projs, hypos, pair_diff=True) if pair_diff else aggregate(feats, ref_proj, src_projs, hypos)
                 if ((not self.training or cost.is_cuda) and getattr(regular, "fused_regress", False)
                         and getattr(self.Depth_regress, "mdf_builtin", False)):
                     prob, depth = regular(cost, hypos)
diff --git a/mdf-net_amd/net/unit/backbone.py b/mdf-net_amd/net/unit/backbone.py
--- a/mdf-net_amd/net/unit/backbone.py
+++ b/mdf-net_amd/net/unit/backbone.py
@@ -11,6 +11,11 @@
 import os as _os
 _HEADS = bool(int(_os.environ.get("MDF_FPN_HEADS_FUSED", "1")))
 _PAIR = bool(int(_os.environ.get("MDF_CONV_PAIR", "1")))
+_PAIR_DIFF = bool(int(_os.environ.get("MDF_PAIR_DIFF", "1")))
+
+
+def pair_difference_rows(w):
+    return w[1::2] - w[0::2]
 
 
 def _stage(cin, cout, first_k, first_s):
@@ -34,32 +39,36 @@
         self.out3 = nn.Conv2d(c3, c2, 1, bias=False)
         self.out4 = nn.Conv2d(c3, c3, 1, bias=False)
 
-    def _composed_heads(self):
+    def _composed_fp64(self, pair_diff=False):
+        def mat(m):
+            return m.weight.detach().double().reshape(m.out_channels, m.in_channels)
+        o2, o3, l2, l3 = mat(self.out2), mat(self.out3), mat(self.lat2), mat(self.lat3)
+        b2, b3 = self.lat2.bias.detach().double(), self.lat3.bias.detach().double()
+        heads = {"y4": (mat(self.out4), None), "a4": (o3, None), "y3": (o3 @ l3, o3 @ b3),
+                 "c4": (o2, None), "c3": (o2 @ l3, o2 @ b3), "y2": (o2 @ l2, o2 @ b2)}
+        if pair_diff:
+            heads = {k: (pair_difference_rows(w), None if b is None else pair_difference_rows(b)) for k, (w, b) in heads.items()}
+        return heads
+
+    def _composed_heads(self, pair_diff=False):
         mods = (self.out2, self.out3, self.out4, self.lat2, self.lat3)
         tensors = [t for m in mods for t in (m.weight, m.bias) if t is not None]
 
         def build():
-            def mat(m):
-                return m.weight.detach().double().reshape(m.out_channels, m.in_channels)
-            o2, o3, l2, l3 = mat(self.out2), mat(self.out3), mat(self.lat2), mat(self.lat3)
-            b2, b3 = self.lat2.bias.detach().double(), self.lat3.bias.detach().double()
-
             def pack(w, bias=None):
                 w4 = w.float().reshape(w.shape[0], w.shape[1], 1, 1).contiguous()
                 return ops.pack_conv2d_weight(w4), (None if bias is None else bias.float().contiguous()), w.shape[1], w.shape[0]
-            return {"y4": pack(mat(self.out4)), "a4": pack(o3), "y3": pack(o3 @ l3, o3 @ b3),
-                    "c4": pack(o2), "c3": pack(o2 @ l3, o2 @ b3), "y2": pack(o2 @ l2, o2 @ b2)}
-        return layers.cache_of(self.out2).get(tensors, build)
+            return {k: pack(w, b) for k, (w, b) in self._composed_fp64(pair_diff).items()}
+        return (layers.cache_of_key(self, "pair_diff_heads") if pair_diff else layers.cache_of(self.out2)).get(tensors, build)
 
-    def _hip_forward(self, x):
+    def _hip_forward(self, x, pair_diff=False):
+        return self._hip_heads(*self._hip_trunk(x), pair_diff=pair_diff)
+
+    def _hip_trunk(self, x):
         def seq(blocks, t):
             for blk in blocks:
                 t = layers.conv2d_layer(blk.conv, blk.bn, t, relu=True)
             return t
-
-        def head(h, t, res_up=None):
-            wp, bias, cin, cout = h
-            return ops.conv2d_nhwc(t, wp, cin, cout, 1, 1, None, bias, False, None, 1.0, res_up)
         with torch.no_grad():
             first, second = self.conv01[0], self.conv01[1]
             xin = x.float().contiguous()
@@ -71,8 +80,16 @@
             t2 = seq(self.conv12, t1)
             t3 = seq(self.conv23, t2)
             t4 = seq(self.conv34, t3)
-            hd = self._composed_heads()
-            if _HEADS and (hd["y4"][2], hd["y4"][3], hd["a4"][3], hd["c4"][3], hd["y3"][2], hd["y3"][3], hd["c3"][2], hd["c3"][3]) == (64, 64, 32, 16, 32, 32, 32, 16) \
+        return t2, t3, t4
+
+    def _hip_heads(self, t2, t3, t4, pair_diff=False):
+        def head(h, t, res_up=None):
+            wp, bias, cin, cout = h
+            return ops.conv2d_nhwc(t, wp, cin, cout, 1, 1, None, bias, False, None, 1.0, res_up)
+        with torch.no_grad():
+            hd = self._composed_heads(pair_diff)
+            built = (64, 32, 16, 8, 32, 16, 32, 8) if pair_diff else (64, 64, 32, 16, 32, 32, 32, 16)
+            if _HEADS and (hd["y4"][2], hd["y4"][3], hd["a4"][3], hd["c4"][3], hd["y3"][2], hd["y3"][3], hd["c3"][2], hd["c3"][3]) == built \
                     and tuple(t3.shape[1:3]) == (2 * t4.shape[1], 2 * t4.shape[2]):
                 y4, a4, c4 = ops.conv1x1_heads(t4, [hd["y4"], hd["a4"], hd["c4"]], [None, None, None])
                 y3, c3 = ops.conv1x1_heads(t3, [hd["y3"], hd["c3"]], [a4, c4])
@@ -104,9 +121,11 @@
             out.append(trip)
         return out
 
-    def forward(self, x: torch.Tensor):
+    def forward(self, x: torch.Tensor, pair_diff: bool = False):
+        if pair_diff and not layers.hip_eval(self, x):
+            raise RuntimeError("pair-difference pyramids exist in eval mode on a GPU only")
         if layers.hip_eval(self, x):
-            return self._hip_forward(x)
+            return self._hip_forward(x, pair_diff)
         if layers.hip_train(self, x):
             from mdfnet_hip import train_ops
             return self._heads(*train_ops.trunk_train(self, x, groups=1))
diff --git a/mdf-net_amd/net/unit/homoaggregate.py b/mdf-net_amd/net/unit/homoaggregate.py
--- a/mdf-net_amd/net/unit/homoaggregate.py
+++ b/mdf-net_amd/net/unit/homoaggregate.py
@@ -24,7 +24,13 @@
         sd = {k: v for k, v in self.depth_weight.state_dict(keep_vars=True).items()}
         return layers.cache_of(self).get(list(sd.values()), lambda: ops.fold_view_weight(sd, self.ngroups, prefix=""))
 
-    def forward(self, features, ref_proj, src_projs, depth_hypos):
+    def forward(self, features, ref_proj, src_projs, depth_hypos, pair_diff=False):
+        if pair_diff:
+            if self.training or any(f.shape[1] != self.ngroups for f in features):
+                raise RuntimeError("pair-difference maps are an eval-mode input with ngroups channels")
+            with torch.no_grad():
+                proj = _projections(ref_proj, src_projs, features[0].device)
+                return ops.warp_aggregate_pairdiff(list(features), proj, depth_hypos, self._params())
         if layers.hip_train(self, *features, depth_hypos):
             from mdfnet_hip import train_ops
             proj = _projections(ref_proj, src_projs, features[0].device)
```

After: 297.9 views/s (median of 6 runs). +6.9%, better.
